# neobotix/neo_mpc_planner2

Measured on AMD Instinct MI355X. Metric: MPC solves/sec (control_steps=3, 500x500 costmap), higher is better.
Workload: dtype f64

## Files before the change

neo_mpc_planner2_amd/csrc/adjoint.h:

```cpp
#pragma once
#include "neo_mpc_device.h"
#include "wave_ops.h"
#include "fast_math.h"
#include "solver_context.h"
#include "costmap.h"
#include "riccati.h"

namespace neo_mpc {
namespace {

template <bool kTame, bool kRiccati, int kFew = 0>
__device__ __forceinline__ void adjoint_by_scans(const SolveArgs& a, const Ctx& c, double* L, bool exact_step, int lane, int n,
                                                 bool& free_path, int& nhops) {
  auto scan = [](double v) { if constexpr (kFew > 0) return wave_scan_few<kFew>(v); else return wave_scan(v); };
  constexpr int kLast = kFew > 0 ? kFew - 1 : 63;
  const DevParams& p = a.p;
  const double* u = L + a.lds.u;
  double* gs = L + a.lds.gs;
  float* RS = reinterpret_cast<float*>(L + a.lds.ric);
  float* ARTF = reinterpret_cast<float*>(L + a.lds.rt);
  const bool on = lane < n;
  const double vx = on ? u[3 * lane] : 0.0, vy = on ? u[3 * lane + 1] : 0.0, w = on ? u[3 * lane + 2] : 0.0;
  const double th = scan(w * p.dt);
  double sn, cs;
  sincos_heading<kTame>(th, &sn, &cs);
  const double ddx = (vx * cs - vy * sn) * p.dt, ddy = (vx * sn + vy * cs) * p.dt;
  const double x = scan(ddx), y = scan(ddy);
  double rt = on ? -2.0 * p.wo_n * (c.tyaw - th) : 0.0;
  if (lane == n - 1) rt += -2.0 * p.wterm_o * (c.fyaw - th);
  const double rx = on ? -2.0 * p.wt_n * (c.cx - x) : 0.0, ry = on ? -2.0 * p.wt_n * (c.cy - y) : 0.0;
  const double px = scan(rx), py = scan(ry);
  const double SX = lane_value(px, kLast) - px + rx, SY = lane_value(py, kLast) - py + ry;
  const double tt = on ? rt - ddy * SX + ddx * SY : 0.0;
  const double pt = scan(tt);
  const double ST = lane_value(pt, kLast) - pt + tt;
  int raw_here = 0;
  bool has_hop = false;
  float hop_x = 0.0f, hop_y = 0.0f;
  if (on) {
    gs[3 * lane] = p.dt * (cs * SX + sn * SY);
    gs[3 * lane + 1] = p.dt * (-sn * SX + cs * SY);
    gs[3 * lane + 2] = p.dt * ST;
    if (kRiccati) {
      float* rs = RS + kRicStage * lane;
      rs[RS_CS] = (float)cs; rs[RS_SN] = (float)sn; rs[RS_PX] = (float)ddx; rs[RS_PY] = (float)ddy;
      double wxx, wxy, wyy, wlx, wly;
      raw_here = edge_stickiness(a, c, L, x, y, cs, sn, wxx, wxy, wyy, wlx, wly, has_hop, hop_x, hop_y);
      rs[RS_WXX] = (float)wxx; rs[RS_WXY] = (float)wxy; rs[RS_WYY] = (float)wyy;
      rs[RS_WLX] = (float)wlx; rs[RS_WLY] = (float)wly;
      rs[RS_SY] = exact_step ? (float)SY : 0.0f;
      ARTF[2 * lane + 1] = exact_step ? (float)SX : 0.0f;
    }
  }
  if (kRiccati) {
    free_path = __ballot(raw_here != 0) == 0ull;
    const unsigned long long hmask = __ballot(has_hop);
    const int rank = __popcll(hmask & ((1ull << lane) - 1ull));
    double* t = L + a.lds.tol;
    if (has_hop && rank < kHopLanes) {
      reinterpret_cast<int*>(t + T_HOP_STAGE)[rank] = lane;
      reinterpret_cast<float*>(t + T_HOP_VEC)[2 * rank] = hop_x;
      reinterpret_cast<float*>(t + T_HOP_VEC)[2 * rank + 1] = hop_y;
    }
    nhops = min(__popcll(hmask), (int)kHopLanes);
    if (lane == 0) reinterpret_cast<int*>(t + T_HOP_STAGE)[kHopLanes] = nhops;
  }
  WAVE_SYNC();
}

template <int kSteps, bool kTame>
__device__ __forceinline__ void adjoint_short_sweep(const SolveArgs& a, const Ctx& c, double* L, bool have_trig, int lane, int n) {
  const DevParams& p = a.p;
  const double* u = L + a.lds.u;
  double* gs = L + a.lds.gs;
  double* ACS = L + a.lds.cs;
  double* ASN = L + a.lds.sn;
  double* ADX = L + a.lds.dxs;
  double* ADY = L + a.lds.dys;
  double* ARX = L + a.lds.rx;
  double* ARY = L + a.lds.ry;
  double* ART = L + a.lds.rt;
  double x = 0.0, y = 0.0, th = 0.0;
#pragma unroll
  for (int i = 0; i < n; ++i) {
    const double vx = u[3 * i], vy = u[3 * i + 1], w = u[3 * i + 2];
    th += w * p.dt;
    double sn, cs;
    if (kSteps && have_trig) { sn = ASN[i]; cs = ACS[i]; }
    else sincos_heading<kTame>(th, &sn, &cs);
    const double ddx = (vx * cs - vy * sn) * p.dt, ddy = (vx * sn + vy * cs) * p.dt;
    x += ddx; y += ddy;
    double rt = -2.0 * p.wo_n * (c.tyaw - th);
    if (i == n - 1) rt += -2.0 * p.wterm_o * (c.fyaw - th);
    if (lane == 0) {
      ACS[i] = cs; ASN[i] = sn; ADX[i] = ddx; ADY[i] = ddy;
      ARX[i] = -2.0 * p.wt_n * (c.cx - x); ARY[i] = -2.0 * p.wt_n * (c.cy - y); ART[i] = rt;
    }
  }
  WAVE_SYNC();
  double SX = 0.0, SY = 0.0, ST = 0.0;
#pragma unroll
  for (int k = n - 1; k >= 0; --k) {
    SX += ARX[k]; SY += ARY[k];
    ST += ART[k] - ADY[k] * SX + ADX[k] * SY;
    if (lane == 0) {
      gs[3 * k] = p.dt * (ACS[k] * SX + ASN[k] * SY);
      gs[3 * k + 1] = p.dt * (-ASN[k] * SX + ACS[k] * SY);
      gs[3 * k + 2] = p.dt * ST;
    }
  }
  WAVE_SYNC();
}

}
}
```

neo_mpc_planner2_amd/csrc/costmap.h:

```cpp
#pragma once
#include <hip/hip_runtime.h>
#include <math.h>
#include <stdint.h>

#include "neo_mpc_device.h"
#include "wave_ops.h"
#include "solver_context.h"
#include "fast_math.h"
#include "solver_rules.h"

namespace neo_mpc {
namespace {

__device__ __forceinline__ int cell_of(double w, double origin, double res, double inv) {
  double t = w - origin;
  double q = t * inv;
  double fl = floor(q);
  if (fabs(q - rint(q)) < 1e-6) fl = floor(t / res);
  int cell;
  asm("v_cvt_i32_f64 %0, %1" : "=v"(cell) : "v"(fl));
  return cell;
}

__device__ __forceinline__ int map_raw(const DevMap& m, int mx, int my) {
  if (mx < -m.border || my < -m.border || mx >= m.size_x + m.border || my >= m.size_y + m.border)
    return 254;
  return m.cells[(long)my * m.pitch + mx];
}

__device__ __forceinline__ int raw_occupancy(int raw) {
  return raw == 0 ? 0 : raw == 253 ? 99 : raw == 254 ? 100 : raw == 255 ? -1 : 1 + (97 * (raw - 1)) / 251;
}
__device__ __forceinline__ double raw_cost(int raw) { return (double)raw_occupancy(raw) / 100.0; }

template <bool kCovered = false>
__device__ __forceinline__ int cell_raw(const SolveArgs& a, const Ctx& c, const double* L, int mx, int my) {
  const unsigned tx = (unsigned)(mx - c.tile_x0), ty = (unsigned)(my - c.tile_y0);
  const int lg = c.tile_geom & 31;
  if (kCovered || ((tx >> lg) == 0u && ty < (unsigned)(c.tile_geom >> 8)))
    return reinterpret_cast<const uint8_t*>(L + a.lds.tile)[(ty << lg) + tx];
  return map_raw(a.map, mx, my);
}

template <bool kCovered = false>
__device__ __forceinline__ double step_term(const SolveArgs& a, const Ctx& c, const double* L, double x, double y) {
  if (c.tile_geom & kTileFree) return L[a.lds.term];
  const double X = c.X0 + (c.c0 * x - c.s0 * y), Y = c.Y0 + (c.s0 * x + c.c0 * y);
  const int mx = cell_of(X, a.map.origin_x, a.map.resolution, a.map.inv_resolution);
  const int my = cell_of(Y, a.map.origin_y, a.map.resolution, a.map.inv_resolution);
  return L[a.lds.term + cell_raw<kCovered>(a, c, L, mx, my)];
}

constexpr double kSticky = NEO_RULE_STICKY, kWall = NEO_RULE_WALL, kStickyDist = NEO_RULE_STICKY_DIST, kWallDist = NEO_RULE_WALL_DIST;
constexpr double kHopMargin = NEO_RULE_HOP_MARGIN;
template <bool kCovered = false>
__device__ __forceinline__ int edge_stickiness(const SolveArgs& a, const Ctx& c, const double* L, double x, double y,
                                               double cs, double sn, double& wxx, double& wxy, double& wyy, double& lx,
                                               double& ly, bool& hop, float& hop_x, float& hop_y) {
  wxx = 0.0; wxy = 0.0; wyy = 0.0; lx = 0.0; ly = 0.0;
  hop = false; hop_x = 0.0f; hop_y = 0.0f;
  if (c.tile_geom & kTileFree) return 0;
  const double X = c.X0 + (c.c0 * x - c.s0 * y), Y = c.Y0 + (c.s0 * x + c.c0 * y);
  const int mx = cell_of(X, a.map.origin_x, a.map.resolution, a.map.inv_resolution);
  const int my = cell_of(Y, a.map.origin_y, a.map.resolution, a.map.inv_resolution);
  const double fx = (X - a.map.origin_x) * a.map.inv_resolution - (double)mx;
  const double fy = (Y - a.map.origin_y) * a.map.inv_resolution - (double)my;
  const int raw_here = cell_raw<kCovered>(a, c, L, mx, my);
  const double here = L[a.lds.term + raw_here];
  const bool far = mx <= -2147483647 || mx >= 2147483646 || my <= -2147483647 || my >= 2147483646;
  if (far) return raw_here;
  const double hop_range = L[a.lds.tol + T_HOP_RANGE];
  const double zone = fmax(kWallDist, hop_range);
  const bool xlo = fx < zone, xhi = 1.0 - fx < zone, ylo = fy < zone, yhi = 1.0 - fy < zone;
  double rx = 0.0, ry = 0.0, pbx = 0.0, pby = 0.0;
  double drop = L[a.lds.tol + T_HOP_DROP], hwx = 0.0, hwy = 0.0;
  if (xlo || xhi) {
    const int raw_n = cell_raw<kCovered>(a, c, L, xlo ? mx - 1 : mx + 1, my);
    const double dist = xlo ? fx : 1.0 - fx, there = L[a.lds.term + raw_n];
    const bool wall = raw_n == 254 && raw_here != 254;
    if (wall) { if (dist < kWallDist) { rx = kWall * 2.0 * a.p.wt_n; pbx = (xlo ? kWallDist - dist : dist - kWallDist) * a.map.resolution; } }
    else if (dist < kStickyDist && there > here) rx = kSticky * 2.0 * a.p.wt_n;
    if (dist < hop_range && here - there > drop) {
      drop = here - there; hop = true;
      hwx = (xlo ? -1.0 : 1.0) * (dist + kHopMargin) * a.map.resolution; hwy = 0.0;
    }
  }
  if (ylo || yhi) {
    const int raw_n = cell_raw<kCovered>(a, c, L, mx, ylo ? my - 1 : my + 1);
    const double dist = ylo ? fy : 1.0 - fy, there = L[a.lds.term + raw_n];
    const bool wall = raw_n == 254 && raw_here != 254;
    if (wall) { if (dist < kWallDist) { ry = kWall * 2.0 * a.p.wt_n; pby = (ylo ? kWallDist - dist : dist - kWallDist) * a.map.resolution; } }
    else if (dist < kStickyDist && there > here) ry = kSticky * 2.0 * a.p.wt_n;
    if (dist < hop_range && here - there > drop) {
      hop = true;
      hwx = 0.0; hwy = (ylo ? -1.0 : 1.0) * (dist + kHopMargin) * a.map.resolution;
    }
  }
  wxx = rx * c.c0 * c.c0 + ry * c.s0 * c.s0;
  wxy = rx * c.c0 * -c.s0 + ry * c.s0 * c.c0;
  wyy = rx * c.s0 * c.s0 + ry * c.c0 * c.c0;
  lx = -(rx * pbx * c.c0 + ry * pby * c.s0);
  ly = -(rx * pbx * -c.s0 + ry * pby * c.c0);
  if (hop) {
    const double hrx = c.c0 * hwx + c.s0 * hwy, hry = -c.s0 * hwx + c.c0 * hwy, idt = rcp_fast(a.p.dt);
    hop_x = (float)((cs * hrx + sn * hry) * idt); hop_y = (float)((-sn * hrx + cs * hry) * idt);
  }
  return raw_here;
}

__device__ double edge_cost(const DevMap& m, double ax, double ay, double bx, double by) {
  int x0 = cell_of(ax, m.origin_x, m.resolution, m.inv_resolution);
  int y0 = cell_of(ay, m.origin_y, m.resolution, m.inv_resolution);
  const int x1 = cell_of(bx, m.origin_x, m.resolution, m.inv_resolution);
  const int y1 = cell_of(by, m.origin_y, m.resolution, m.inv_resolution);
  if (x0 < 0 || y0 < 0 || x0 >= m.size_x || y0 >= m.size_y || x1 < 0 || y1 < 0 || x1 >= m.size_x || y1 >= m.size_y)
    return raw_cost(254);
  const long dx = labs((long)x1 - x0), dy = labs((long)y1 - y0);
  const int sx = x1 >= x0 ? 1 : -1, sy = y1 >= y0 ? 1 : -1;
  long err = dx - dy;
  double worst = -1.0;
  for (long guard = 0; guard <= dx + dy + 1; ++guard) {
    worst = fmax(worst, raw_cost(map_raw(m, x0, y0)));
    if (x0 == x1 && y0 == y1) break;
    long e2 = 2 * err;
    if (e2 > -dy) { err -= dy; x0 += sx; }
    if (e2 < dx) { err += dx; y0 += sy; }
  }
  return worst;
}

__device__ double footprint_cost(const SolveArgs& a, const double* L, uint32_t b, int lane) {
  if (!a.footprints || a.footprint_points == 0) return L[a.lds.prob + P_FOOTPRINT];
  const int np = (int)a.footprint_points;
  const double* pts = a.footprints + (size_t)b * 2 * np;
  double worst = -1.0;
  for (int e = lane; e < np; e += kLanes) {
    int j = (e + 1) % np;
    worst = fmax(worst, edge_cost(a.map, pts[2 * e], pts[2 * e + 1], pts[2 * j], pts[2 * j + 1]));
  }
  return wave_max(worst);
}

}
}
```

neo_mpc_planner2_amd/csrc/feasible_set.h:

```cpp
#pragma once
#include <hip/hip_runtime.h>
#include <math.h>
#include <stdint.h>

#include "neo_mpc_device.h"
#include "fast_math.h"
#include "solver_context.h"

namespace neo_mpc {
namespace {

__device__ __forceinline__ double clampd(double v, double lo, double hi) { return v < lo ? lo : (v > hi ? hi : v); }

template <bool kTame = false>
__device__ __forceinline__ void project_block(const DevParams& p, double& b0, double& b1, double& b2) {
  b2 = fmin(fmax(b2, p.lo[2]), p.hi[2]);
  const double zx = b0, zy = b1, r = p.r;
  if (kTame || p.disc_in_box) {
    const double n2 = zx * zx + zy * zy;
    if (n2 > r * r) { const double sc = r * rsq_fast1(n2); b0 = zx * sc; b1 = zy * sc; }
    return;
  }
  const double px = clampd(zx, p.lo[0], p.hi[0]), py = clampd(zy, p.lo[1], p.hi[1]);
  if (px * px + py * py <= r * r) { b0 = px; b1 = py; return; }
  const double nz = sqrt(zx * zx + zy * zy);
  const double qx = zx * (r / nz), qy = zy * (r / nz);
  if (qx >= p.lo[0] && qx <= p.hi[0] && qy >= p.lo[1] && qy <= p.hi[1]) { b0 = qx; b1 = qy; return; }
  double best = INFINITY, bx = px, by = py;
  for (int e = 0; e < 4; ++e) {
    const double fixed = (e == 0) ? p.lo[0] : (e == 1) ? p.hi[0] : (e == 2) ? p.lo[1] : p.hi[1];
    if (fabs(fixed) > r) continue;
    const double o = sqrt(r * r - fixed * fixed);
    for (int s = -1; s <= 1; s += 2) {
      const double ex = (e < 2) ? fixed : s * o, ey = (e < 2) ? s * o : fixed;
      if (ex < p.lo[0] || ex > p.hi[0] || ey < p.lo[1] || ey > p.hi[1]) continue;
      const double dd = (ex - zx) * (ex - zx) + (ey - zy) * (ey - zy);
      if (dd < best) { best = dd; bx = ex; by = ey; }
    }
  }
  b0 = bx; b1 = by;
}

#define NEO_QN_STEPS                                                                                  \
  1.0, 0.84, 1.19, 0.71, 1.41, 0.59, 1.68, 0.5, 2.0, 0.42, 2.38, 0.35, 2.83, 0.25, 4.0, 0.177,         \
  0.125, 0.088, 0.0625, 0.044, 0.03125, 0.0156, 0.0078, 0.0039, 0.00195, 0.00098, 4.9e-4, 2.4e-4,    \
  1.2e-4, 6e-5, 3e-5, 1.5e-5
__constant__ double kQnSteps[32] = {NEO_QN_STEPS};
constexpr unsigned long long newton_lanes_at_least(double t) {
  constexpr double steps[32] = {NEO_QN_STEPS};
  unsigned long long m = 0;
  for (int l = 32; l < 64; ++l) {
    const double s = l >= 61 ? (double)(1 << (l - 58)) : steps[l - 32];
    if (s >= t) m |= 1ull << l;
  }
  return m;
}
constexpr unsigned long long kNewtonLanes = 0xffffffff00000000ull;

template <bool kLongShots>
__device__ __forceinline__ double lane_scale(int lane) {
  if (kLongShots && lane >= 61) return ldexp(1.0, lane - 58);
  if (lane >= 32) return kQnSteps[lane - 32];
  double s = ldexp(1.0, -12 + (lane >> 1));
  return (lane & 1) ? s * 1.4142135623730951 : s;
}

template <bool kTame = false, bool kRiccati = false>
__device__ __forceinline__ void candidate_block(const SolveArgs& a, const Ctx& c, const double* L, int lane,
                                                double step, double pstep, int i, double& b0, double& b1,
                                                double& b2, int hop_stage = -1, float hop_x = 0.0f, float hop_y = 0.0f) {
  const double* u = L + a.lds.u + 3 * i;
  if (kRiccati && hop_stage >= 0) {
    b0 = u[0]; b1 = u[1]; b2 = u[2];
    if (i == hop_stage) { b0 += (double)hop_x; b1 += (double)hop_y; project_block<kTame>(a.p, b0, b1, b2); }
    return;
  }
  const int* am = reinterpret_cast<const int*>(L + a.lds.mode) + 4 * i;
  const bool near = am[2] != 0;
  if (near && lane >= 32 && (lane & 1)) { b0 = u[0]; b1 = u[1]; b2 = u[2]; return; }
  if (lane < 32 || near) {
    if (lane >= 32) step = pstep;
    if (kRiccati) step *= (double)a.p.n * rcp_fast((double)(a.p.n - i));
    const double* gs = L + a.lds.gs + 3 * i;
    const double e0 = (u[0] - step * gs[0]) - c.v0, e1 = (u[1] - step * gs[1]) - c.v1,
                 e2 = (u[2] - step * gs[2]) - c.v2;
    const double ne2 = e0 * e0 + e1 * e1 + e2 * e2;
    const double sh = (ne2 > 0.0) ? fmax(0.0, 1.0 - step * a.p.wc_n * rsq_fast1(ne2)) : 0.0;
    b0 = c.v0 + sh * e0; b1 = c.v1 + sh * e1; b2 = c.v2 + sh * e2;
  } else {
    const double* d = L + a.lds.d + 3 * i;
    if (kRiccati && am[3]) {
      if (step >= 1.0) { b0 = c.v0; b1 = c.v1; b2 = c.v2; }
      else { b0 = u[0] + step * d[0]; b1 = u[1] + step * d[1]; b2 = u[2] + step * d[2]; }
    } else {
      b0 = u[0] + step * d[0]; b1 = u[1] + step * d[1]; b2 = u[2] + step * d[2];
      const double rl = a.p.r * (1.0 - 1e-12);
      if (!kTame && !a.p.disc_in_box && am[0] == 1 && !(am[1] & 2) && u[0] * u[0] + u[1] * u[1] < rl * rl) {
        const double nxb = L[a.lds.nx + i];
        const double fixed = nxb != 0.0 ? u[0] : u[1];
        const double lim2 = a.p.r * a.p.r - fixed * fixed, lim = lim2 > 0.0 ? sqrt(lim2) * (1.0 - 1e-15) : 0.0;
        if (nxb != 0.0) { b0 = fixed; b1 = clampd(b1, -lim, lim); }
        else { b1 = fixed; b0 = clampd(b0, -lim, lim); }
      }
    }
  }
  project_block<kTame>(a.p, b0, b1, b2);
}

}
}
```

neo_mpc_planner2_amd/csrc/k1_solve.h:

```cpp
#pragma once
#include <hip/hip_runtime.h>
#include <hip/hip_ext.h>
#include <math.h>
#include <stdint.h>
#include <stdlib.h>

#include "neo_mpc_device.h"
#include "wave_ops.h"
#include "fast_math.h"
#include "solver_context.h"
#include "solver_rules.h"
#include "costmap.h"
#include "feasible_set.h"
#include "rollout.h"
#include "riccati.h"
#include "adjoint.h"
#include "tangent_cone.h"
#include "dense_newton.h"
#include "lbfgs.h"
#include "cell_scan.h"
#include "k1_timing.h"

namespace neo_mpc {
namespace {

constexpr int kStallIterations = NEO_RULE_STALL_ITERATIONS;
constexpr int kBlockedRun = NEO_RULE_BLOCKED_RUN;
constexpr double kBlockedStep = NEO_RULE_BLOCKED_STEP;
constexpr double kFinalFracGaussNewton = NEO_RULE_FINAL_FRAC_GN;
constexpr double kWindowStep = NEO_RULE_WINDOW_STEP;
constexpr int kClosingRun = NEO_RULE_CLOSING_RUN;
constexpr int kLateIteration = NEO_RULE_LATE_ITERATION;
constexpr int kNewtonMaxSteps = 8;

constexpr int kRoutedSteps = 3;
constexpr LdsLayout make_routed_stagewise_layout() {
  LdsLayout l = make_lds_layout(kRoutedSteps, 0, true, true);
  constexpr LdsLayout dense = make_lds_layout(kRoutedSteps, 4, false);
  l.tile = dense.tile;
  l.total_bytes = dense.total_bytes;
  return l;
}
static_assert(make_lds_layout(kRoutedSteps, 0, true, true).tile <= make_lds_layout(kRoutedSteps, 4, false).tile,
              "the stage-wise arrays of three stages fit in front of the dense kernel's reach tile");
static_assert(make_lds_layout(kRoutedSteps, 0, true, true).gr == make_lds_layout(kRoutedSteps, 4, false).gr,
              "records, iterate and gradients share their offsets");
template <int kSteps, int kStaticTile, int kLayoutSteps, bool kRouted = false>
__device__ __forceinline__ void fresh_args(SolveArgs& a) {
  auto kp = (const __attribute__((address_space(4))) char*)__builtin_amdgcn_kernarg_segment_ptr();
  asm volatile("" : "+s"(kp));
  a = *(const SolveArgs*)kp;
  if (kRouted) {
    constexpr LdsLayout kLayout = make_routed_stagewise_layout();
    const int tile_w = a.lds.tile_w, tile_h = a.lds.tile_h, reach = a.lds.reach;
    a.lds = kLayout;
    a.lds.tile_w = tile_w; a.lds.tile_h = tile_h; a.lds.reach = reach;
    a.p.n = kRoutedSteps;
  } else if (kSteps || kStaticTile) {
    constexpr LdsLayout kStaticLayout = make_lds_layout(kLayoutSteps, kSteps ? 4 : 0, false);
    const int tile_w = a.lds.tile_w, tile_h = a.lds.tile_h, reach = a.lds.reach;
    a.lds = kStaticLayout;
    a.lds.tile_w = tile_w; a.lds.tile_h = tile_h; a.lds.reach = reach;
    if (kSteps) a.p.n = kSteps;
  }
}
__device__ __forceinline__ void own_loop_params(SolveArgs& a) {
  auto own = [](double& v) { asm volatile("" : "+s"(v)); };
  own(a.p.dt); own(a.p.wt_n); own(a.p.wo_n); own(a.p.wc_n); own(a.p.wterm_o); own(a.p.r);
  own(a.p.lo[2]); own(a.p.hi[2]);
  own(a.map.origin_x); own(a.map.origin_y); own(a.map.resolution); own(a.map.inv_resolution);
}
template <bool kVectorPose>
__device__ __forceinline__ void ctx_from_lds(const SolveArgs& a, const double* L, Ctx& c) {
  const double* P = L + a.lds.prob;
  const double* t = L + a.lds.tol;
  c.cx = lane_value(P[P_CARROT_X], 0); c.cy = lane_value(P[P_CARROT_Y], 0);
  c.tyaw = lane_value(t[T_TYAW], 0); c.fyaw = lane_value(t[T_FYAW], 0);
  c.v0 = lane_value(P[P_VEL], 0); c.v1 = lane_value(P[P_VEL + 1], 0); c.v2 = lane_value(P[P_VEL + 2], 0);
  c.c0 = t[T_C0]; c.s0 = t[T_S0]; c.X0 = P[P_CUR_X]; c.Y0 = P[P_CUR_Y];
  if (kVectorPose) asm volatile("" : "+v"(c.c0), "+v"(c.s0), "+v"(c.X0), "+v"(c.Y0));
  else { c.c0 = lane_value(c.c0, 0); c.s0 = lane_value(c.s0, 0); c.X0 = lane_value(c.X0, 0); c.Y0 = lane_value(c.Y0, 0); }
  const int* ti = reinterpret_cast<const int*>(t + T_TILE);
  c.tile_x0 = uniform_int(ti[0]); c.tile_y0 = uniform_int(ti[1]); c.tile_geom = uniform_int(ti[2]);
  c.konst = 0.0; c.true_yaw = 0.0;
}

struct SolveCarry {
  int flags;
  bool cold;
  bool wall_in_reach;
  double f = INFINITY;
  int it = 0, nfev = 1, status = NEO_MPC_STATUS_MAX_ITER;
};

template <int kSteps, bool kTame, int kStaticTile, int kLayoutSteps>
__device__ __forceinline__ bool solve_setup(double* L, uint32_t b, int lane, SolveCarry& s) {
  constexpr bool kCovered = kStaticTile > 0;
  int flags;
  bool cold = true;
  {
    SolveArgs a;
    fresh_args<kSteps, kStaticTile, kLayoutSteps>(a);
    const DevParams& p = a.p;
    const int n = kSteps ? kSteps : p.n, nv = 3 * n;
    load_records(a, L, b, lane);
    if (uniform_int(reinterpret_cast<const int*>(L + a.lds.prob)[PI_SKIP]) == 1) { skip_instance(a, b, lane); return false; }
    select_map(a.map, L + a.lds.prob);
    flags = reset_and_warm(a, L, b, lane) ? NEO_MPC_FLAG_RESET : 0;
    const double fcost = footprint_cost(a, L, b, lane);
    if (lane == 0) L[a.lds.prob + P_FOOTPRINT] = fcost;
    Ctx c;
    make_ctx_wave(p, a.map, L + a.lds.prob, fcost, c, lane);
    load_tile(a, c, L, lane);
    s.wall_in_reach = (c.tile_geom & kTileWall) != 0;
    if (s.wall_in_reach) flags |= NEO_MPC_FLAG_WALL_IN_REACH;
    if (lane == 0) {
      double* t = L + a.lds.tol;
      t[T_XTOL] = p.xtol; t[T_EARLY] = p.early_tol; t[T_FINAL] = p.final_tol; t[T_FTOL] = p.ftol;
      t[T_STALL] = p.stall_step; t[T_WTOL] = p.wtol; t[T_WTOL_LATE] = p.wtol_late; t[T_KINK] = p.kink_radius;
      t[T_KONST] = c.konst; t[T_TRUE_YAW] = c.true_yaw;
      t[T_HOP_DROP] = p.hop_min_drop; t[T_HOP_RANGE] = p.hop_range;
      t[T_BTOL_MAP] = p.btol_map; t[T_BTOL_FREE] = p.btol_free;
      reinterpret_cast<int*>(t + T_HOP_STAGE)[kHopLanes] = 0;
      t[T_C0] = c.c0; t[T_S0] = c.s0; t[T_TYAW] = c.tyaw; t[T_FYAW] = c.fyaw;
      int* ti = reinterpret_cast<int*>(t + T_TILE);
      ti[0] = c.tile_x0; ti[1] = c.tile_y0; ti[2] = c.tile_geom;
    }
    double* u = L + a.lds.u;
    for (int i = lane; i < n; i += kLanes) project_block<kTame>(p, u[3 * i], u[3 * i + 1], u[3 * i + 2]);
    WAVE_SYNC();
    for (int k = 0; k < nv; ++k) cold = cold && (u[k] == 0.0);
    ctx_from_lds<false>(a, L, c);
    {
      double* S = L + a.lds.state;
      int* Si = reinterpret_cast<int*>(S);
      const bool has_prev = uniform_int(Si[SI_HAS_PREV]) == 1 && !(flags & NEO_MPC_FLAG_RESET);
      WAVE_SYNC();
      if (lane == 0) {
        double q0 = has_prev ? S[S_PREV_U0] : u[nv - 3], q1 = has_prev ? S[S_PREV_U0 + 1] : u[nv - 2], q2 = has_prev ? S[S_PREV_U0 + 2] : u[nv - 1];
        project_block<kTame>(p, q0, q1, q2);
        S[S_PREV_U0] = q0; S[S_PREV_U0 + 1] = q1; S[S_PREV_U0 + 2] = q2;
        Si[SI_HAS_PREV] = 0;
      }
      WAVE_SYNC();
    }
    if (!cold && n > 1 && !(p.compat & kCompatNoUnshift) && p.max_it < kDumpGradient) {
      const double* A0 = L + a.lds.state + S_PREV_U0;
      double ts = 0.0;
      const double fs = rollout_cost<kSteps, kTame, kCovered>(
          a, c, L,
          [&](int i, double& b0, double& b1, double& b2) {
            const double* src = lane == 1 ? (i == 0 ? A0 : u + 3 * (i - 1)) : u + 3 * i;
            b0 = src[0]; b1 = src[1]; b2 = src[2];
          },
          NoRecord(), &ts);
      const double f_warm = lane_value(fs, 0), f_alt = lane_value(fs, 1);
      const bool free_both = lane_value(ts, 0) == 0.0 && lane_value(ts, 1) == 0.0;
      if (f_alt < f_warm && free_both) {
        double v0 = 0.0, v1 = 0.0, v2 = 0.0;
        const int k0 = lane, k1 = lane + kLanes, k2 = lane + 2 * kLanes;
        if (k0 < nv) v0 = k0 >= 3 ? u[k0 - 3] : A0[k0];
        if (k1 < nv) v1 = u[k1 - 3];
        if (k2 < nv) v2 = u[k2 - 3];
        WAVE_SYNC();
        if (k0 < nv) u[k0] = v0;
        if (k1 < nv) u[k1] = v1;
        if (k2 < nv) u[k2] = v2;
      } else if (f_alt < f_warm && lane == 0) {
        reinterpret_cast<int*>(L + a.lds.state)[SI_HAS_PREV] = kAltArmed;
      }
      WAVE_SYNC();
    }
  }
  s.flags = flags; s.cold = cold;
  return true;
}

template <int kMinWavesPerSimd, int kSteps, int kDir, bool kTame, int kStaticTile, int kLayoutSteps, bool kRouted = false>
__device__ __forceinline__ bool solve_search(double* L, uint32_t b, SolveCarry& sc) {
  constexpr bool kCovered = kStaticTile > 0;
  constexpr bool kNewton = kDir == 1;
  constexpr bool kRiccati = kDir == 2;
  constexpr bool kSecond = kDir != 0;
  constexpr bool kBlockedRule = kNewton || kRouted;
  static_assert(!kRiccati || kSteps == 0 || kRouted, "the stage-wise direction: run-time-sized, or the routed kernel's control_steps-3 branch");
  static_assert(!kRouted || (kRiccati && kSteps == kRoutedSteps), "the routed branch is the stage-wise one, three stages in registers");
  constexpr int kFew = (kRiccati && kSteps > 0) ? kSteps : 0;
  constexpr int kNwSteps = !kNewton ? 1 : kSteps ? kSteps : kNewtonMaxSteps;
  constexpr bool kVectorPose = kTame;
  constexpr int kRegSteps = kSteps ? kSteps : 1;
  constexpr int kPairs = kSteps ? 4 : NEO_MPC_MAX_LBFGS_MEMORY;
  double f = sc.f;
  const bool cold = sc.cold;
  int npairs = 0, head = 0, nfev = sc.nfev, it = sc.it, status = sc.status, stall = 0;
  int blocked_run = 0;
  int nblocked = 1;
  double u_term = 0.0;
  double gain1 = INFINITY, gain2 = INFINITY;
  bool final_step = false;
  double alpha = 1.0;
  bool scanned = false;
  int nscans = 0;
  bool scan_only = false;
  auto lane_again = []() {
    int zero;
    asm volatile("v_mov_b32 %0, 0" : "=v"(zero));
    return (int)__builtin_amdgcn_mbcnt_hi(~0u, __builtin_amdgcn_mbcnt_lo(~0u, (unsigned)zero));
  };
  NEO_SEGMENT_DECL;
  NEO_SEGMENT(0);
  for (;;) {
  SolveArgs a;
  fresh_args<kSteps, kStaticTile, kLayoutSteps, kRouted>(a);
  own_loop_params(a);
  select_map(a.map, L + a.lds.prob);
  const DevParams& p = a.p;
  const int n = kSteps ? kSteps : p.n, nv = 3 * n, mem = p.mem;
  double cand[3 * kRegSteps], cand_sn[kRegSteps], cand_cs[kRegSteps];
  bool have_trig = false;
  Ctx c;
  ctx_from_lds<kVectorPose>(a, L, c);
  double* u = L + a.lds.u;
  double* gs = L + a.lds.gs;
  double* gt = L + a.lds.gt;
  double* gr = L + a.lds.gr;
  double* d = L + a.lds.d;
  double* u_prev = L + a.lds.u_prev;
  double* gt_prev = L + a.lds.gt_prev;
  double* u_new = L + a.lds.u_new;
  double* ACS = L + a.lds.cs;
  double* ASN = L + a.lds.sn;
  int* AMODE = reinterpret_cast<int*>(L + a.lds.mode);
  static_assert(2 * 7 >= kNewtonRecord, "Newton records do not fit the step arrays");

  if (!scanned && nscans == 0) {
    const int lane = lane_again();
    for (int i = lane; i < n; i += kLanes) { AMODE[4 * i + 2] = 0; AMODE[4 * i + 3] = 0; }
    if (kRouted && lane == 0) L[a.lds.tol + T_KINK] = p.kink_radius_stagewise;
    alpha = kRiccati ? fmax(1.0, n * 0.125) : 1.0;
    if (kFew && lane == 0) { double* t = L + a.lds.tol; t[T_GAIN1] = INFINITY; t[T_GAIN2] = INFINITY; t[T_ALPHA] = alpha; }
    if (kRiccati && lane == 0) L[a.lds.tol + T_MU] = n > 8 ? (double)(n - 8) * 0.125 : 0.0;
  }
  bool v_feasible = false;
  if (kRiccati) {
    double b0 = c.v0, b1 = c.v1, b2 = c.v2;
    asm volatile("" : "+v"(b0), "+v"(b1), "+v"(b2));
    project_block<kTame>(p, b0, b1, b2);
    v_feasible = b0 == c.v0 && b1 == c.v1 && b2 == c.v2;
  }
  double my_scale;
  {
    int l0 = lane_again();
    my_scale = kRiccati ? 0.0 : lane_scale<kSecond>(l0);
  }
  for (; it < p.max_it && !scan_only; ++it) {
    int lane = lane_again();
    const bool exact_step = kRiccati && nblocked == 0;
    int tol_off = a.lds.tol;
    asm volatile("" : "+s"(tol_off));
    const double* TOL = L + tol_off;
    NEO_PHASE_DECL;
    NEO_PHASE(0);
    constexpr int kVars = 3 * kNwSteps;
    const int nvr = kSteps ? kVars : nv;
    bool free_path = false;
    int nhops = 0;
    float hc[kVars];
    float newton_sol = 0.0f;
    if (kNewton) {
      double hcol[kSteps ? kVars : 1];
      const double hstep = 1e-6, inv_h = 1.0 / hstep;
      double pcs[kNwSteps], psn[kNwSteps];
      double x = 0.0, y = 0.0, th = 0.0;
    #pragma unroll
      for (int i = 0; i < kNwSteps; ++i) {
        if (kSteps || i < n) {
          const double vx = u[3 * i] + (lane == 3 * i ? hstep : 0.0);
          const double vy = u[3 * i + 1] + (lane == 3 * i + 1 ? hstep : 0.0);
          const double w = u[3 * i + 2] + (lane == 3 * i + 2 ? hstep : 0.0);
          th += w * p.dt;
          sincos_heading<kTame>(th, &psn[i], &pcs[i]);
          x += (vx * pcs[i] - vy * psn[i]) * p.dt;
          y += (vx * psn[i] + vy * pcs[i]) * p.dt;
        }
      }
      double SX = 0.0, SY = 0.0, ST = 0.0;
    #pragma unroll
      for (int k = kNwSteps - 1; k >= 0; --k) {
        if (kSteps || k < n) {
          const double vx = u[3 * k] + (lane == 3 * k ? hstep : 0.0);
          const double vy = u[3 * k + 1] + (lane == 3 * k + 1 ? hstep : 0.0);
          const double w = u[3 * k + 2] + (lane == 3 * k + 2 ? hstep : 0.0);
          const double pdx = (vx * pcs[k] - vy * psn[k]) * p.dt, pdy = (vx * psn[k] + vy * pcs[k]) * p.dt;
          double prt = -2.0 * p.wo_n * (c.tyaw - th);
          if (k == n - 1) prt += -2.0 * p.wterm_o * (c.fyaw - th);
          SX += -2.0 * p.wt_n * (c.cx - x); SY += -2.0 * p.wt_n * (c.cy - y);
          ST += prt - pdy * SX + pdx * SY;
          const double g0 = p.dt * (pcs[k] * SX + psn[k] * SY), g1 = p.dt * (-psn[k] * SX + pcs[k] * SY),
                       g2 = p.dt * ST;
          if (kSteps) {
            hcol[3 * k] = g0; hcol[3 * k + 1] = g1; hcol[3 * k + 2] = g2;
          } else {
            const double b0 = lane_value(g0, 63), b1 = lane_value(g1, 63), b2 = lane_value(g2, 63);
            if (lane == 63) { gs[3 * k] = b0; gs[3 * k + 1] = b1; gs[3 * k + 2] = b2; }
            hc[3 * k] = (float)((g0 - b0) * inv_h);
            hc[3 * k + 1] = (float)((g1 - b1) * inv_h);
            hc[3 * k + 2] = (float)((g2 - b2) * inv_h);
          }
          x -= pdx; y -= pdy; th -= w * p.dt;
        } else {
          hc[3 * k] = 0.0f; hc[3 * k + 1] = 0.0f; hc[3 * k + 2] = 0.0f;
        }
      }
      if (kSteps) {
    #pragma unroll
        for (int j = 0; j < kVars; ++j) {
          const double base = lane_value(hcol[j], 63);
          if (lane == 63) gs[j] = base;
          hc[j] = (float)((hcol[j] - base) * inv_h);
        }
      }
      WAVE_SYNC();
    }
    else if (!kSteps || kRiccati) adjoint_by_scans<kTame, kRiccati, kFew>(a, c, L, exact_step, lane, n, free_path, nhops);
    else adjoint_short_sweep<kSteps, kTame>(a, c, L, have_trig, lane, n);
    NEO_PHASE(1);
    const bool my_corner = tangent_cone_pass<kTame, kNewton, kRiccati>(a, c, L, TOL[T_KINK], lane, n);
    WAVE_SYNC();
    const bool corner_any = kSecond && !kTame && __ballot(my_corner) != 0ull && (kRiccati ? free_path : (it > 0 && u_term == 0.0));
    NEO_PHASE(2);
    if (p.max_it == kDumpGradient) {
      for (int k = lane; k < nv; k += kLanes) a.solution[(size_t)b * nv + k] = gt[k];
      return true;
    }
    if (kSecond && it == 0 && cold) {
      if (kRiccati) { for (int k = lane; k < nv; k += kLanes) d[k] = -gr[k]; }
      else if (lane < nvr) d[lane] = -gr[lane];
      if (kRiccati) for (int i = lane; i < n; i += kLanes) AMODE[4 * i + 3] = 0;
      WAVE_SYNC();
    } else if (kRiccati) {
      riccati_prepare(a, c, L, n, lane, v_feasible, (float)TOL[T_MU]);
      WAVE_SYNC();
      if (corner_any) riccati_keep_linear_terms(a, L, n, lane, true);
      auto sweep = [&]() {
        riccati_sweep<float, (kMinWavesPerSimd < 4), kFew>(a, L, n, lane);
        riccati_finish(a, c, L, n, lane);
      };
      sweep();
      if (!kTame && corner_any && repin_corner_blocks<true>(a, L, n, lane)) {
        riccati_keep_linear_terms(a, L, n, lane, false);
        sweep();
      }
    } else if (kNewton) {
      newton_sol = dense_newton_direction<kSteps, kNwSteps, kTame>(a, L, hc, corner_any, lane, n, nvr);
    }
    NEO_PHASE(3);
    if (!kSecond) lbfgs_direction<kSteps, kPairs>(a, L, it, mem, head, npairs, lane, n);
    if (kSecond && it > 0) {
      float dm = 0.0f;
      int anynear = 0;
      if (kRiccati) {
        for (int k = lane; k < nv; k += kLanes) {
          const float v = (float)fabs(d[k]);
          dm = (v == v) ? fmaxf(dm, v) : INFINITY;
          anynear |= (AMODE[4 * (k / 3) + 2] == 1);
        }
      } else if (lane < nvr) { dm = fabsf(newton_sol); anynear = (AMODE[4 * (lane / 3) + 2] == 1); }
      dm = wave_max_f(dm);
      const bool near_any = __ballot(anynear != 0) != 0ull;
      if ((double)dm < TOL[T_EARLY] && !near_any && nhops == 0) { status = NEO_MPC_STATUS_CONVERGED; break; }
      if ((double)dm < ((kRiccati && !exact_step) ? kFinalFracGaussNewton : 1.0) * TOL[T_FINAL] && !near_any) final_step = true;
    }
    NEO_PHASE(4);
    if (p.max_it > kDumpGradient && it == p.max_it - kDumpGradient - 1) {
      for (int k = lane; k < nv; k += kLanes) a.solution[(size_t)b * nv + k] = d[k];
      return true;
    }
    const double lscale = kRiccati ? lane_scale<kSecond>(lane) : my_scale;
    const double alpha_now = kFew ? TOL[T_ALPHA] : alpha;
    const double pstep = alpha_now * lscale;
    const double step = lane < 32 ? pstep : lscale;
    bool took_trial = false;
    double fb = INFINITY, cterm = 0.0;
    int best = 32;
    if (kRiccati && free_path && it > 0) took_trial = riccati_free_space_trial<kTame, kCovered, kFew, kBlockedRule>(a, c, L, n, lane, alpha_now, f, fb, cterm);
    const double* ALT0 = L + a.lds.state + S_PREV_U0;
    bool alt_armed = false;
    if (it == 0) alt_armed = uniform_int(reinterpret_cast<const int*>(L + a.lds.state)[SI_HAS_PREV]) == kAltArmed;
    if (!took_trial) {
    int hop_stage = -1;
    float hop_x = 0.0f, hop_y = 0.0f;
    if (kRiccati && lane >= 1 && lane <= nhops) {
      const double* t = TOL;
      hop_stage = reinterpret_cast<const int*>(t + T_HOP_STAGE)[lane - 1];
      hop_x = reinterpret_cast<const float*>(t + T_HOP_VEC)[2 * (lane - 1)];
      hop_y = reinterpret_cast<const float*>(t + T_HOP_VEC)[2 * (lane - 1) + 1];
    }
    double fc = rollout_cost<kSteps, kTame, kCovered>(
        a, c, L,
        [&](int i, double& b0, double& b1, double& b2) {
          candidate_block<kTame, kRiccati>(a, c, L, lane, step, pstep, i, b0, b1, b2, hop_stage, hop_x, hop_y);
          if (it == 0) {
            asm volatile("");
            if (lane == 0) { b0 = u[3 * i]; b1 = u[3 * i + 1]; b2 = u[3 * i + 2]; }
            if (lane == kAltLane && alt_armed) { const double* src = i == 0 ? ALT0 : u + 3 * (i - 1); b0 = src[0]; b1 = src[1]; b2 = src[2]; }
          }
          if (kSteps) { cand[3 * i] = b0; cand[3 * i + 1] = b1; cand[3 * i + 2] = b2; }
        },
        [&](int i, double sn, double cs) {
          if (kSteps && !kSecond) { cand_sn[i] = sn; cand_cs[i] = cs; }
        }, kBlockedRule ? &cterm : nullptr);
    NEO_PHASE(5);
    if (!(fc == fc)) fc = INFINITY;
    if (it == 0) { f = lane_value(fc, 0); if (kNewton) u_term = lane_value(cterm, 0); }
    fb = fc;
    best = lane;
    wave_argmin(fb, best);
    }
    ++nfev;
    if (!(fb < f)) { status = NEO_MPC_STATUS_CONVERGED; ++it; break; }
    const bool alt_won = alt_armed && best == kAltLane;
    float stepmax = 0.0f;
    if (kSteps && kSecond && !took_trial) {
      if (lane == best) {
#pragma unroll
        for (int k = 0; k < 3 * kRegSteps; ++k) {
          stepmax = fmaxf(stepmax, (float)fabs(cand[k] - u[k]));
          u[k] = cand[k];
        }
      }
      stepmax = __builtin_bit_cast(float, __builtin_amdgcn_readlane(__builtin_bit_cast(int, stepmax), best));
      have_trig = true;
    } else {
      if (kSteps && !kSecond) {
        if (lane == best) {
#pragma unroll
          for (int i = 0; i < kRegSteps; ++i) {
            u_new[3 * i] = cand[3 * i]; u_new[3 * i + 1] = cand[3 * i + 1]; u_new[3 * i + 2] = cand[3 * i + 2];
            ASN[i] = cand_sn[i]; ACS[i] = cand_cs[i];
          }
        }
      } else if (!kSteps && !took_trial) {
        const double bstep = lane_value(step, best), bpstep = lane_value(pstep, best);
        int bhop = -1;
        float bhx = 0.0f, bhy = 0.0f;
        if (kRiccati && best >= 1 && best <= nhops) {
          bhop = reinterpret_cast<const int*>(TOL + T_HOP_STAGE)[best - 1];
          bhx = reinterpret_cast<const float*>(TOL + T_HOP_VEC)[2 * (best - 1)];
          bhy = reinterpret_cast<const float*>(TOL + T_HOP_VEC)[2 * (best - 1) + 1];
        }
        for (int i = lane; i < n; i += kLanes) {
          double b0, b1, b2;
          candidate_block<kTame, kRiccati>(a, c, L, best, bstep, bpstep, i, b0, b1, b2, bhop, bhx, bhy);
          if (alt_won) { const double* src = i == 0 ? ALT0 : u + 3 * (i - 1); b0 = src[0]; b1 = src[1]; b2 = src[2]; }
          u_new[3 * i] = b0; u_new[3 * i + 1] = b1; u_new[3 * i + 2] = b2;
        }
      }
      have_trig = true;
      WAVE_SYNC();
      for (int k = lane; k < nv; k += kLanes) {
        const double nu = u_new[k], ou = u[k];
        stepmax = fmaxf(stepmax, (float)fabs(nu - ou));
        if (!kSecond) { u_prev[k] = ou; gt_prev[k] = gt[k]; }
        u[k] = nu;
      }
      stepmax = wave_max_f(stepmax);
    }
    const double gain = f - fb;
    const double fscale = fmax(1.0, fabs(fb));
    stall = (gain <= TOL[T_FTOL] * fscale || (double)stepmax <= TOL[T_STALL]) ? stall + 1 : 0;
    const bool hop_won = (kRiccati && best >= 1 && best <= nhops) || alt_won;
    nblocked = (best < 32 || lane_value(step, best) < kWindowStep || hop_won) ? nblocked + 1 : 0;
    const bool window_on = !kRiccati || kRouted || nblocked >= 3;
    const double wtol0 = TOL[T_WTOL];
    const double wtol = it >= kLateIteration ? TOL[T_WTOL_LATE] : wtol0;
    const double g1 = kFew ? TOL[T_GAIN1] : gain1, g2 = kFew ? TOL[T_GAIN2] : gain2;
    bool creeping = wtol > 0.0 && gain + g1 + g2 <= wtol * fscale && window_on;
    bool free_now = kRiccati ? free_path : false;
    if (kNewton) free_now = lane_value(cterm, best) == 0.0;
    creeping = creeping || (wtol0 > 0.0 && (double)stepmax <= TOL[T_STALL] && gain <= 0.5 * g1 && g1 <= 0.5 * g2 &&
                            (!free_now || (g2 < INFINITY && gain * gain <= TOL[T_FTOL] * fscale * (g1 - gain))) &&
                            ((kRiccati && !kRouted) ? window_on : nblocked >= kClosingRun));
    bool blocked_stop = false;
    if (kBlockedRule) {
      const double bs = lane_value(step, best);
      blocked_run = (best < 32 || bs < kBlockedStep) ? blocked_run + 1 : 0;
      if (blocked_run >= kBlockedRun) {
        const bool free_rollout = lane_value(cterm, best) == 0.0;
        const double btol = free_rollout ? TOL[T_BTOL_FREE] : TOL[T_BTOL_MAP];
        blocked_stop = gain + g1 + g2 <= btol;
      }
    }
    double* TOLW = L + tol_off;
    if (kFew) { if (lane == 0) { TOLW[T_GAIN2] = g1; TOLW[T_GAIN1] = gain; } }
    else { gain2 = gain1; gain1 = gain; }
    f = fb;
    if (nblocked != 0) final_step = false;
    if (kNewton) u_term = lane_value(cterm, best);
    if (kRiccati && !(it == 0 && cold) && !hop_won) {
      constexpr unsigned long long kNearlyFull = newton_lanes_at_least(0.8), kShort = kNewtonLanes & ~newton_lanes_at_least(0.3);
      const double mu0 = n > 8 ? (double)(n - 8) * 0.125 : 0.0, mu = TOL[T_MU];
      double* mu_slot = L + tol_off + T_MU;
      if ((kNearlyFull >> best) & 1ull) { if (lane == 0) *mu_slot = fmax(0.25 * mu, mu0 * 0.0625); }
      else if (best < 32 || ((kShort >> best) & 1ull)) { if (lane == 0) *mu_slot = fmin(4.0 * mu, 16.0 * mu0); }
    }
    if (best < 32 && !hop_won) {
      const double al = clampd(lane_value(step, best), 1e-6, 1e6);
      if (kFew) { if (lane == 0) TOLW[T_ALPHA] = al; }
      else alpha = al;
    }
    WAVE_SYNC();
    NEO_PHASE(6);
    NEO_PHASE_DUMP();
    if ((double)stepmax < TOL[T_XTOL] || stall >= kStallIterations || creeping || final_step || blocked_stop) { status = NEO_MPC_STATUS_CONVERGED; ++it; break; }
  }

  if (!kSecond || scanned || status != NEO_MPC_STATUS_CONVERGED || p.max_it >= kDumpGradient) break;
  const bool nothing_to_scan = (c.tile_geom & kTileFree) || (kNewton && u_term == 0.0);
  if (nothing_to_scan && nscans == 0) break;
  bool resume = false;
  {
    SolveArgs as;
    fresh_args<kSteps, kStaticTile, kLayoutSteps, kRouted>(as);
    select_map(as.map, L + as.lds.prob);
    Ctx cs;
    ctx_from_lds<false>(as, L, cs);
    int ls = lane_again();
    if (nscans == 0 && ls == 0) L[as.lds.tol + T_FSCAN] = f;
    NEO_SEGMENT_SCAN_BEGIN();
    const bool w = !nothing_to_scan &&
                   cell_scan<kSteps, kTame, kCovered>(as, cs, L, f, kNewton ? &u_term : nullptr, nfev, ls, kSteps ? kSteps : as.p.n);
    NEO_SEGMENT_SCAN_END();
    ++nscans;
    scan_only = w && nscans < NEO_RULE_SCAN_REPEATS;
    if (!scan_only) {
      scanned = true;
      WAVE_SYNC();
      resume = L[as.lds.tol + T_FSCAN] - f > as.p.scan_resume_gain && it < as.p.max_it;
      if (kFew && resume) {
        if (ls == 0) { L[as.lds.tol + T_GAIN1] = INFINITY; L[as.lds.tol + T_GAIN2] = INFINITY; }
        WAVE_SYNC();
      }
    }
  }
  if (scan_only) continue;
  if (!resume) break;
  status = NEO_MPC_STATUS_MAX_ITER; stall = 0; final_step = false; blocked_run = 0; nblocked = 1;
  gain1 = INFINITY; gain2 = INFINITY;
  }
  NEO_SEGMENT(1);
  NEO_SEGMENT_DUMP();
  if (scanned && status == NEO_MPC_STATUS_MAX_ITER) status = NEO_MPC_STATUS_CONVERGED;
  sc.f = f; sc.it = it; sc.nfev = nfev; sc.status = status;
  return false;
}

template <int kSteps, int kStaticTile, int kLayoutSteps>
__device__ __forceinline__ void solve_finish(double* L, uint32_t b, int lane, const SolveCarry& sc) {
  const int flags = sc.flags, status = sc.status, it = sc.it, nfev = sc.nfev;
  double f = sc.f;
  SolveArgs a;
  fresh_args<kSteps, kStaticTile, kLayoutSteps>(a);
  select_map(a.map, L + a.lds.prob);
  const DevParams& p = a.p;
  const int n = kSteps ? kSteps : p.n, nv = 3 * n;
  double* u = L + a.lds.u;
  Ctx c;
  ctx_from_lds<false>(a, L, c);
#ifndef NEO_MPC_PHASE_TIMING
  if (a.solution && p.max_it < kDumpGradient)
    for (int k = lane; k < nv; k += kLanes) a.solution[(size_t)b * nv + k] = u[k];
#endif
  WAVE_SYNC();
  f += L[a.lds.tol + T_KONST];
  c.true_yaw = L[a.lds.tol + T_TRUE_YAW];
  postprocess(a, c, L, b, lane, u, status == NEO_MPC_STATUS_CONVERGED, L[a.lds.prob + P_FOOTPRINT], flags, f, status, it, nfev);
}

template <int kMinWavesPerSimd, int kSteps, int kDir = 0, bool kTame = false, int kStaticTile = 0>
__global__ __launch_bounds__(kLanes, kMinWavesPerSimd) void k_solve(const SolveArgs args) {
  extern __shared__ __align__(16) double Ldyn[];
  constexpr int kLayoutSteps = kSteps ? kSteps : kNewtonMaxSteps;
  constexpr LdsLayout kStaticLayout = make_lds_layout(kLayoutSteps, kSteps ? 4 : 0, false);
  constexpr int kStaticDoubles = kStaticTile ? (kStaticLayout.total_bytes + kStaticTile) / 8 : 2;
  __shared__ __align__(16) double Lstat[kStaticDoubles];
  double* const L = kStaticTile ? Lstat : Ldyn;
  const int lane = threadIdx.x;
  if (blockIdx.x >= args.count) return;
  const uint32_t b = args.order ? (uint32_t)__builtin_amdgcn_readfirstlane((int)args.order[blockIdx.x]) : blockIdx.x;
  if (b >= args.count) return;
  NEO_WAVE_START;
  SolveCarry sc;
  if (!solve_setup<kSteps, kTame, kStaticTile, kLayoutSteps>(L, b, lane, sc)) return;
  if (solve_search<kMinWavesPerSimd, kSteps, kDir, kTame, kStaticTile, kLayoutSteps>(L, b, sc)) return;
  solve_finish<kSteps, kStaticTile, kLayoutSteps>(L, b, lane, sc);
  NEO_WAVE_END_ARGS(args);
}

template <int kMinWavesPerSimd, bool kTame = false, int kStaticTile = 0>
__global__ __launch_bounds__(kLanes, kMinWavesPerSimd) void k_solve_routed(const SolveArgs args) {
  extern __shared__ __align__(16) double Ldyn[];
  constexpr int kSteps = kRoutedSteps;
  constexpr LdsLayout kStaticLayout = make_lds_layout(kSteps, 4, false);
  constexpr int kStaticDoubles = kStaticTile ? (kStaticLayout.total_bytes + kStaticTile) / 8 : 2;
  __shared__ __align__(16) double Lstat[kStaticDoubles];
  double* const L = kStaticTile ? Lstat : Ldyn;
  const int lane = threadIdx.x;
  if (blockIdx.x >= args.count) return;
  const uint32_t b = args.order ? (uint32_t)__builtin_amdgcn_readfirstlane((int)args.order[blockIdx.x]) : blockIdx.x;
  if (b >= args.count) return;
  NEO_WAVE_START;
  SolveCarry sc;
  if (!solve_setup<kSteps, kTame, kStaticTile, kSteps>(L, b, lane, sc)) return;
  if (__builtin_amdgcn_readfirstlane((int)sc.wall_in_reach)) {
    __builtin_amdgcn_s_setprio(3);
    if (solve_search<kMinWavesPerSimd, kSteps, 2, kTame, kStaticTile, kSteps, true>(L, b, sc)) return;
  } else {
    if (solve_search<kMinWavesPerSimd, kSteps, 1, kTame, kStaticTile, kSteps, false>(L, b, sc)) return;
  }
  solve_finish<kSteps, kStaticTile, kSteps>(L, b, lane, sc);
  NEO_WAVE_END_ARGS(args);
}

int solve_variant(const LaunchTuning& t, int fallback) { return t.solve_waves ? t.solve_waves : fallback; }

using SolveKernel = void (*)(const SolveArgs);
void launch_k1(SolveKernel kernel, size_t lds_bytes, const SolveArgs& a, void* stream, void* ev_start, void* ev_stop) {
  const dim3 grid(a.count), block(kLanes);
  hipEvent_t e0 = (hipEvent_t)ev_start, e1 = (hipEvent_t)ev_stop;
  if (e0 || e1) hipExtLaunchKernelGGL(kernel, grid, block, lds_bytes, (hipStream_t)stream, e0, e1, 0, a);
  else hipLaunchKernelGGL(kernel, grid, block, lds_bytes, (hipStream_t)stream, a);
}
#define NEO_K1_BY_WAVES(w, kernel, ...) \
  ((w) == 4 ? (SolveKernel)kernel<4, __VA_ARGS__> : (w) == 3 ? (SolveKernel)kernel<3, __VA_ARGS__> : (SolveKernel)kernel<2, __VA_ARGS__>)

}
}
```

neo_mpc_planner2_amd/csrc/k1_timing.h:

```cpp
#pragma once

#ifdef NEO_MPC_PHASE_TIMING
#ifdef NEO_MPC_SEGMENT_TIMING
#define NEO_SEGMENT_DECL unsigned long long seg_t0 = 0, seg_t1 = 0, seg_scan = 0, seg_scan_at = 0
#define NEO_SEGMENT(k) seg_t##k = wall_clock64()
#define NEO_SEGMENT_SCAN_BEGIN() seg_scan_at = wall_clock64(); seg_scan = seg_scan_at
#define NEO_SEGMENT_SCAN_END() seg_scan = wall_clock64() - seg_scan
#define NEO_SEGMENT_DUMP()                                                                                   \
  {                                                                                                          \
    SolveArgs ad;                                                                                            \
    fresh_args<kSteps, kStaticTile, kLayoutSteps, kRouted>(ad);                                              \
    const int nvd = 3 * ad.p.n;                                                                              \
    if (ad.solution && lane_again() == 0 && nvd >= 9) {                                                      \
      ad.solution[(size_t)b * nvd + 4] = (double)seg_t0; ad.solution[(size_t)b * nvd + 5] = (double)seg_t1;  \
      ad.solution[(size_t)b * nvd + 3] = (double)seg_scan; ad.solution[(size_t)b * nvd + 2] = (double)seg_scan_at; \
    }                                                                                                        \
  }
#else
#define NEO_SEGMENT_DECL
#define NEO_SEGMENT(k)
#define NEO_SEGMENT_SCAN_BEGIN()
#define NEO_SEGMENT_SCAN_END()
#define NEO_SEGMENT_DUMP()
#endif
#define NEO_WAVE_START const unsigned long long wave_t0 = wall_clock64()
#define NEO_WAVE_END_ARGS(args)                                                                     \
  if ((args).solution && lane == 0 && (args).p.n >= 3) {                                            \
    const int nvw = 3 * (args).p.n;                                                                \
    unsigned int hw_id, xcc_id;                                                                    \
    asm volatile("s_getreg_b32 %0, hwreg(HW_REG_HW_ID)" : "=s"(hw_id));                            \
    asm volatile("s_getreg_b32 %0, hwreg(HW_REG_XCC_ID)" : "=s"(xcc_id));                          \
    (args).solution[(size_t)b * nvw + 6] = (double)wave_t0;                                        \
    (args).solution[(size_t)b * nvw + 7] = (double)wall_clock64();                                 \
    (args).solution[(size_t)b * nvw + 8] = (double)hw_id + 4294967296.0 * (double)(xcc_id & 15u);  \
  }
#define NEO_PHASE_DECL long long phase_clock[8]
#define NEO_PHASE(k) phase_clock[k] = clock64()
#define NEO_PHASE_DUMP()                                                                            \
  if (it == 2 && a.solution && lane == 0)                                                          \
    for (int k = 0; k < 6; ++k) a.solution[(size_t)b * nv + k] = (double)(phase_clock[k + 1] - phase_clock[k])
#else
#define NEO_WAVE_START
#define NEO_WAVE_END_ARGS(args)
#define NEO_SEGMENT_DECL
#define NEO_SEGMENT(k)
#define NEO_SEGMENT_SCAN_BEGIN()
#define NEO_SEGMENT_SCAN_END()
#define NEO_SEGMENT_DUMP()
#define NEO_PHASE_DECL
#define NEO_PHASE(k)
#define NEO_PHASE_DUMP()
#endif
```

neo_mpc_planner2_amd/csrc/riccati.h:

```cpp
#pragma once
#include <hip/hip_runtime.h>
#include <math.h>
#include <stdint.h>

#include "neo_mpc_device.h"
#include "wave_ops.h"
#include "fast_math.h"
#include "solver_context.h"
#include "solver_rules.h"
#include "costmap.h"
#include "feasible_set.h"

namespace neo_mpc {
namespace {

enum : int {
  RS_PX = 0, RS_PY, RS_TX, RS_TY,
  RS_WXX, RS_WXY, RS_WYY, RS_FLAGS,
  RS_C00, RS_C01, RS_C02, RS_C11,
  RS_C12, RS_C22, RS_CS, RS_SN,
  RS_GT = 16,
  RS_GS = 19,
  RS_WK = 22,
  RS_WLX = 25, RS_WLY,
  RS_SY = 27,
  RS_GAIN = 16,
  kRicStage = 28
};
enum : int { RC_FREE3 = 0, RC_SLIDE_W, RC_XY, RC_SLIDE, RC_W, RC_NONE, RC_KINK, RF_CASE = 7, RF_KINK_OK = 8 };

typedef float ric_f4 __attribute__((ext_vector_type(4)));

__device__ __forceinline__ float ric_rcp(float x) { return __builtin_amdgcn_rcpf(x); }
__device__ __forceinline__ double ric_rcp(double x) { return rcp_fast(x); }
template <typename T> __device__ __forceinline__ T ric_max(T a, T b) { return a > b ? a : b; }
template <typename T> __device__ __forceinline__ T ric_abs(T a) { return a < (T)0 ? -a : a; }
__device__ __forceinline__ float ric_fma(float a, float b, float c) { return fmaf(a, b, c); }
__device__ __forceinline__ double ric_fma(double a, double b, double c) { return fma(a, b, c); }
template <typename T> __device__ __forceinline__ T ric_pivot(T p, T delta) { return p > delta ? p : ric_max(ric_abs(p), delta); }

__device__ __forceinline__ void riccati_prepare(const SolveArgs& a, const Ctx& c, double* L, int n, int lane,
                                                bool v_feasible, float mu) {
  if (lane >= n) return;
  const DevParams& p = a.p;
  float* rs = reinterpret_cast<float*>(L + a.lds.ric) + kRicStage * lane;
  const int* am = reinterpret_cast<const int*>(L + a.lds.mode) + 4 * lane;
  const double* gt = L + a.lds.gt + 3 * lane;
  const double* gs = L + a.lds.gs + 3 * lane;
  const double* u = L + a.lds.u + 3 * lane;
  const double cs = rs[RS_CS], sn = rs[RS_SN];
  const double idt = rcp_fast(p.dt);
  rs[RS_GT] = (float)((cs * gt[0] - sn * gt[1]) * idt); rs[RS_GT + 1] = (float)((sn * gt[0] + cs * gt[1]) * idt);
  rs[RS_GT + 2] = (float)(gt[2] * idt);
  rs[RS_GS] = (float)((cs * gs[0] - sn * gs[1]) * idt); rs[RS_GS + 1] = (float)((sn * gs[0] + cs * gs[1]) * idt);
  rs[RS_GS + 2] = (float)(gs[2] * idt);
  const double e0 = u[0] - c.v0, e1 = u[1] - c.v1, e2 = u[2] - c.v2;
  rs[RS_WK] = (float)(-(cs * e0 - sn * e1) * p.dt); rs[RS_WK + 1] = (float)(-(sn * e0 + cs * e1) * p.dt);
  rs[RS_WK + 2] = (float)(-e2 * p.dt);
  const double nx = L[a.lds.nx + lane], ny = L[a.lds.ny + lane];
  const double tx = -ny, ty = nx;
  const float rtx = (float)(cs * tx - sn * ty), rty = (float)(sn * tx + cs * ty);
  rs[RS_TX] = rtx; rs[RS_TY] = rty;
  const int near = am[2];
  const int xy = near ? 2 : am[0];
  const bool wfree = !(near || (am[1] & 1));
  const int kase = xy == 0 ? (wfree ? RC_FREE3 : RC_XY) : xy == 1 ? (wfree ? RC_SLIDE_W : RC_SLIDE) : (wfree ? RC_W : RC_NONE);
  const int flags = kase | ((!near && v_feasible) ? RF_KINK_OK : 0);
  rs[RS_FLAGS] = (float)flags;
  float c00 = 0.0f, c01 = 0.0f, c02 = 0.0f, c11 = 0.0f, c12 = 0.0f, c22 = 0.0f;
  if (!near) {
    const float f0 = (float)(cs * e0 - sn * e1), f1 = (float)(sn * e0 + cs * e1), f2 = (float)e2;
    const float fn2 = f0 * f0 + f1 * f1 + f2 * f2;
    const float ine = fn2 > 0.0f ? __builtin_amdgcn_rsqf(fn2) : 0.0f;
    const float i2 = (float)(idt * idt);
    const float sN = (float)p.wc_n * ine * i2, h0 = f0 * ine, h1 = f1 * ine, h2 = f2 * ine;
    const float k2 = reinterpret_cast<const float*>(L + a.lds.rt)[2 * lane] * i2;
    c00 = sN * (1.0f - h0 * h0) + k2 * rtx * rtx; c01 = -sN * h0 * h1 + k2 * rtx * rty; c02 = -sN * h0 * h2;
    c11 = sN * (1.0f - h1 * h1) + k2 * rty * rty; c12 = -sN * h1 * h2; c22 = sN * (1.0f - h2 * h2);
    const float mt = mu * (float)(2.0 * p.wt_n);
    c00 += mt; c11 += mt; c22 += mu * (float)(2.0 * p.wo_n);
  }
  rs[RS_C00] = c00; rs[RS_C01] = c01; rs[RS_C02] = c02; rs[RS_C11] = c11; rs[RS_C12] = c12; rs[RS_C22] = c22;
}

__device__ __forceinline__ void riccati_keep_linear_terms(const SolveArgs& a, double* L, int n, int lane, bool save) {
  ric_f4* rec = reinterpret_cast<ric_f4*>(reinterpret_cast<float*>(L + a.lds.ric) + kRicStage * lane + RS_GAIN);
  ric_f4* keep = reinterpret_cast<ric_f4*>(L + a.lds.keep) + 3 * lane;
  for (int i = lane; i < n; i += kLanes, rec += 7 * kLanes, keep += 3 * kLanes) {
    if (save) { keep[0] = rec[0]; keep[1] = rec[1]; keep[2] = rec[2]; }
    else { rec[0] = keep[0]; rec[1] = keep[1]; rec[2] = keep[2]; }
  }
  WAVE_SYNC();
}

template <typename T, bool kPrefetch = true, int kFew = 0>
__device__ __forceinline__ void riccati_sweep(const SolveArgs& a, double* L, int n, int lane) {
  const DevParams& p = a.p;
  float* RS = static_cast<float*>(__builtin_assume_aligned(reinterpret_cast<float*>(L + a.lds.ric), 16));
  int* AMODE = reinterpret_cast<int*>(L + a.lds.mode);
  double* d = L + a.lds.d;
  const float* ARTF = reinterpret_cast<const float*>(L + a.lds.rt);
  const T w2 = (T)(2.0 * p.wt_n), wo2 = (T)(2.0 * p.wo_n), wterm2 = (T)(2.0 * p.wterm_o);
  const T wc2 = (T)((p.wc_n * p.wc_n) / (p.dt * p.dt));

  T V00 = (T)0.0, V01 = (T)0.0, V02 = (T)0.0, V11 = (T)0.0, V12 = (T)0.0, V22 = (T)0.0, v0 = (T)0.0, v1 = (T)0.0, v2 = (T)0.0;
  ric_f4 r0, r1, r2, r3, r4, r5, r6;
  if (kPrefetch) {
    const ric_f4* R4 = reinterpret_cast<const ric_f4*>(RS + kRicStage * (n - 1));
    r0 = R4[0]; r1 = R4[1]; r2 = R4[2]; r3 = R4[3]; r4 = R4[4]; r5 = R4[5]; r6 = R4[6];
  }
  for (int i = (kFew ? kFew : n) - 1; i >= 0; --i) {
    const bool first = kFew > 0 && i == 0;
    if (!kPrefetch) {
      const ric_f4* R4 = reinterpret_cast<const ric_f4*>(RS + kRicStage * i);
      r0 = R4[0]; r1 = R4[1]; r2 = R4[2]; r3 = R4[3]; r4 = R4[4]; r5 = R4[5]; r6 = R4[6];
    }
    const T px = r0.x, py = r0.y, rtx = r0.z, rty = r0.w;
    const T wxx = r1.x, wxy = r1.y, wyy = r1.z;
    const int flags = __builtin_amdgcn_readfirstlane((int)r1.w);
    const T c00 = r2.x, c01 = r2.y, c02 = r2.z, c11 = r2.w, c12 = r3.x, c22 = r3.y;
    const T gt0 = r4.x, gt1 = r4.y, gt2 = r4.z, gs0 = r4.w, gs1 = r5.x, gs2 = r5.y, e0 = r5.z, e1 = r5.w, e2 = r6.x;
    v0 += (T)r6.y; v1 += (T)r6.z;
    const T sy = (T)r6.w, sx = (T)ARTF[2 * i + 1];
    if (kPrefetch && i > 0) {
      const ric_f4* R4 = reinterpret_cast<const ric_f4*>(RS + kRicStage * (i - 1));
      r0 = R4[0]; r1 = R4[1]; r2 = R4[2]; r3 = R4[3]; r4 = R4[4]; r5 = R4[5]; r6 = R4[6];
    }
    const T S00 = V00 + w2 + wxx, S01 = V01 + wxy, S11 = V11 + w2 + wyy;
    const T S22 = V22 + wo2 + (i == n - 1 ? wterm2 : (T)0.0);
    const T M02 = ric_fma(-py, S00, ric_fma(px, S01, V02));
    const T M12 = ric_fma(-py, S01, ric_fma(px, S11, V12));
    const T M22 = ric_fma(-py, M02, ric_fma(px, M12, ric_fma(-py, V02, ric_fma(px, V12, S22))));
    const T Z02 = M02 + sy, Z12 = M12 - sx, Z22 = M22 - ric_fma(sx, px, sy * py);
    const T z0 = v0, z1 = v1, z2 = ric_fma(-py, v0, ric_fma(px, v1, v2));
    T k0 = (T)0.0, k1 = (T)0.0, k2 = (T)0.0, K00 = (T)0.0, K01 = (T)0.0, K02 = (T)0.0, K10 = (T)0.0, K11 = (T)0.0, K12 = (T)0.0,
      K20 = (T)0.0, K21 = (T)0.0, K22 = (T)0.0;
    bool tokink = false;
    int kase = flags & RF_CASE;
    if (flags & RF_KINK_OK) {
      const T q0 = gs0 + z0 + S00 * e0 + S01 * e1 + Z02 * e2;
      const T q1 = gs1 + z1 + S01 * e0 + S11 * e1 + Z12 * e2;
      const T q2 = gs2 + z2 + Z02 * e0 + Z12 * e1 + Z22 * e2;
      if (__builtin_amdgcn_readfirstlane((int)(q0 * q0 + q1 * q1 + q2 * q2 <= wc2))) { tokink = true; kase = RC_KINK; }
    }
    const T q0 = gt0 + z0, q1 = gt1 + z1, q2 = gt2 + z2;
    switch (kase) {
      case RC_FREE3: {
        const T Q00 = S00 + c00, Q01 = S01 + c01, Q02 = Z02 + c02, Q11 = S11 + c11, Q12 = Z12 + c12, Q22 = Z22 + c22;
        const T delta = ric_max((T)1e-6 * ric_max(ric_abs(Q00), ric_max(ric_abs(Q11), ric_abs(Q22))), (T)1e-30);
        const T d0 = ric_pivot(Q00, delta), i0 = ric_rcp(d0);
        const T l10 = Q01 * i0, l20 = Q02 * i0;
        const T d1 = ric_pivot(Q11 - l10 * Q01, delta), i1 = ric_rcp(d1);
        const T h12 = Q12 - l20 * Q01;
        const T l21 = h12 * i1;
        const T d2 = ric_pivot(Q22 - l20 * Q02 - l21 * h12, delta), i2 = ric_rcp(d2);
#define NEO_RIC_SOLVE3(r0_, r1_, r2_, x0_, x1_, x2_)                                           \
        {                                                                                        \
          const T y0 = -(r0_), y1 = -(r1_) - l10 * y0, y2 = -(r2_) - l20 * y0 - l21 * y1;        \
          x2_ = y2 * i2;                                                                         \
          x1_ = y1 * i1 - l21 * x2_;                                                             \
          x0_ = y0 * i0 - l10 * x1_ - l20 * x2_;                                                 \
        }
        NEO_RIC_SOLVE3(q0, q1, q2, k0, k1, k2)
        if (first) break;
        NEO_RIC_SOLVE3(S00, S01, M02, K00, K10, K20)
        NEO_RIC_SOLVE3(S01, S11, M12, K01, K11, K21)
        NEO_RIC_SOLVE3(Z02, Z12, Z22, K02, K12, K22)
#undef NEO_RIC_SOLVE3
        v0 = z0 + S00 * k0 + S01 * k1 + M02 * k2;
        v1 = z1 + S01 * k0 + S11 * k1 + M12 * k2;
        v2 = z2 + Z02 * k0 + Z12 * k1 + Z22 * k2;
        V00 = S00 + S00 * K00 + S01 * K10 + M02 * K20;
        V01 = S01 + S00 * K01 + S01 * K11 + M02 * K21;
        V02 = M02 + S00 * K02 + S01 * K12 + M02 * K22;
        V11 = S11 + S01 * K01 + S11 * K11 + M12 * K21;
        V12 = M12 + S01 * K02 + S11 * K12 + M12 * K22;
        V22 = Z22 + Z02 * K02 + Z12 * K12 + Z22 * K22;
        break;
      }
      case RC_SLIDE_W:
      case RC_XY: {
        const bool bw = kase == RC_SLIDE_W;
        const T ax = bw ? rtx : (T)1.0, ay = bw ? rty : (T)0.0;
        const T Q00 = S00 + c00, Q01 = S01 + c01, Q11 = S11 + c11;
        const T Qa0 = ax * Q00 + ay * Q01, Qa1 = ax * Q01 + ay * Q11;
        const T haa = Qa0 * ax + Qa1 * ay;
        const T hab = bw ? ax * (Z02 + c02) + ay * (Z12 + c12) : Qa1;
        const T hbb = bw ? Z22 + c22 : Q11;
        const T ga = ax * q0 + ay * q1, gb = bw ? q2 : q1;
        const T Za0 = ax * S00 + ay * S01, Za1 = ax * S01 + ay * S11, Za2 = ax * Z02 + ay * Z12;
        const T Zb0 = bw ? M02 : S01, Zb1 = bw ? M12 : S11, Zb2 = bw ? Z22 : Z12;
        const T delta = ric_max((T)1e-6 * ric_max(ric_abs(haa), ric_abs(hbb)), (T)1e-30);
        const T d0 = ric_pivot(haa, delta), i0 = ric_rcp(d0);
        const T l = hab * i0;
        const T d1 = ric_pivot(hbb - l * hab, delta), i1 = ric_rcp(d1);
        T ka, kb, Ka0, Ka1, Ka2, Kb0, Kb1, Kb2;
#define NEO_RIC_SOLVE2(ra_, rb_, xa_, xb_)                       \
        {                                                          \
          const T y0 = -(ra_), y1 = -(rb_) - l * y0;               \
          xb_ = y1 * i1;                                           \
          xa_ = y0 * i0 - l * xb_;                                 \
        }
        NEO_RIC_SOLVE2(ga, gb, ka, kb)
        if (first) {
          k0 = ax * ka; k1 = ay * ka;
          if (bw) k2 = kb; else k1 = kb;
          break;
        }
        NEO_RIC_SOLVE2(Za0, Zb0, Ka0, Kb0)
        NEO_RIC_SOLVE2(Za1, Zb1, Ka1, Kb1)
        NEO_RIC_SOLVE2(Za2, Zb2, Ka2, Kb2)
#undef NEO_RIC_SOLVE2
        v0 = z0 + Za0 * ka + Zb0 * kb; v1 = z1 + Za1 * ka + Zb1 * kb; v2 = z2 + Za2 * ka + Zb2 * kb;
        V00 = S00 + Za0 * Ka0 + Zb0 * Kb0; V01 = S01 + Za0 * Ka1 + Zb0 * Kb1; V02 = M02 + Za0 * Ka2 + Zb0 * Kb2;
        V11 = S11 + Za1 * Ka1 + Zb1 * Kb1; V12 = M12 + Za1 * Ka2 + Zb1 * Kb2; V22 = Z22 + Za2 * Ka2 + Zb2 * Kb2;
        k0 = ax * ka; k1 = ay * ka; K00 = ax * Ka0; K01 = ax * Ka1; K02 = ax * Ka2; K10 = ay * Ka0; K11 = ay * Ka1; K12 = ay * Ka2;
        if (bw) { k2 = kb; K20 = Kb0; K21 = Kb1; K22 = Kb2; }
        else { k1 = kb; K10 = Kb0; K11 = Kb1; K12 = Kb2; }
        break;
      }
      case RC_SLIDE: {
        const T Q00 = S00 + c00, Q01 = S01 + c01, Q11 = S11 + c11;
        const T haa = (rtx * Q00 + rty * Q01) * rtx + (rtx * Q01 + rty * Q11) * rty;
        const T i0 = -ric_rcp(ric_pivot(haa, ric_max((T)1e-6 * ric_abs(haa), (T)1e-30)));
        const T Za0 = rtx * S00 + rty * S01, Za1 = rtx * S01 + rty * S11, Za2 = rtx * Z02 + rty * Z12;
        const T ka = (rtx * q0 + rty * q1) * i0, Ka0 = Za0 * i0, Ka1 = Za1 * i0, Ka2 = Za2 * i0;
        if (first) { k0 = rtx * ka; k1 = rty * ka; break; }
        v0 = z0 + Za0 * ka; v1 = z1 + Za1 * ka; v2 = z2 + Za2 * ka;
        V00 = S00 + Za0 * Ka0; V01 = S01 + Za0 * Ka1; V02 = M02 + Za0 * Ka2;
        V11 = S11 + Za1 * Ka1; V12 = M12 + Za1 * Ka2; V22 = Z22 + Za2 * Ka2;
        k0 = rtx * ka; k1 = rty * ka; K00 = rtx * Ka0; K01 = rtx * Ka1; K02 = rtx * Ka2; K10 = rty * Ka0; K11 = rty * Ka1; K12 = rty * Ka2;
        break;
      }
      case RC_W: {
        const T hbb = Z22 + c22;
        const T i0 = -ric_rcp(ric_pivot(hbb, ric_max((T)1e-6 * ric_abs(hbb), (T)1e-30)));
        k2 = q2 * i0;
        if (first) break;
        K20 = M02 * i0; K21 = M12 * i0; K22 = Z22 * i0;
        v0 = z0 + M02 * k2; v1 = z1 + M12 * k2; v2 = z2 + Z22 * k2;
        V00 = S00 + M02 * K20; V01 = S01 + M02 * K21; V02 = M02 + M02 * K22;
        V11 = S11 + M12 * K21; V12 = M12 + M12 * K22; V22 = Z22 + Z22 * K22;
        break;
      }
      case RC_KINK:
        k0 = e0; k1 = e1; k2 = e2;
        if (first) break;
        v0 = z0 + S00 * k0 + S01 * k1 + M02 * k2;
        v1 = z1 + S01 * k0 + S11 * k1 + M12 * k2;
        v2 = z2 + Z02 * k0 + Z12 * k1 + Z22 * k2;
        V00 = S00; V01 = S01; V02 = M02; V11 = S11; V12 = M12; V22 = Z22;
        break;
      default:
        v0 = z0; v1 = z1; v2 = z2;
        V00 = S00; V01 = S01; V02 = M02; V11 = S11; V12 = M12; V22 = Z22;
        break;
    }
    if (lane == 0) {
      ric_f4* G4 = reinterpret_cast<ric_f4*>(RS + kRicStage * i + RS_GAIN);
      G4[0] = ric_f4{(float)K00, (float)K01, (float)K02, (float)K10};
      G4[1] = ric_f4{(float)K11, (float)K12, (float)K20, (float)K21};
      G4[2] = ric_f4{(float)K22, (float)k0, (float)k1, (float)k2};
      AMODE[4 * i + 3] = tokink ? 1 : 0;
    }
  }
  WAVE_SYNC();
  T z0 = (T)0.0, z1 = (T)0.0, z2 = (T)0.0;
  for (int i = 0; i < n; ++i) {
    const ric_f4* R4 = reinterpret_cast<const ric_f4*>(RS + kRicStage * i);
    const ric_f4 s0 = R4[0], g0 = R4[4], g1 = R4[5], g2 = R4[6];
    const T w0 = (T)g2.y + (T)g0.x * z0 + (T)g0.y * z1 + (T)g0.z * z2;
    const T w1 = (T)g2.z + (T)g0.w * z0 + (T)g1.x * z1 + (T)g1.y * z2;
    const T w2f = (T)g2.w + (T)g1.z * z0 + (T)g1.w * z1 + (T)g2.x * z2;
    if (lane == 0) { d[3 * i] = (double)w0; d[3 * i + 1] = (double)w1; d[3 * i + 2] = (double)w2f; }
    const T e0 = z0 + w0, e1 = z1 + w1, e2 = z2 + w2f;
    z0 = ric_fma(-(T)s0.y, e2, e0); z1 = ric_fma((T)s0.x, e2, e1); z2 = e2;
  }
  WAVE_SYNC();
}

__device__ __forceinline__ void riccati_finish(const SolveArgs& a, const Ctx& c, double* L, int n, int lane) {
  if (lane < n) {
    const float* rs = reinterpret_cast<const float*>(L + a.lds.ric) + kRicStage * lane;
    const int* am = reinterpret_cast<const int*>(L + a.lds.mode) + 4 * lane;
    double* d = L + a.lds.d + 3 * lane;
    if (am[3]) {
      const double* u = L + a.lds.u + 3 * lane;
      d[0] = c.v0 - u[0]; d[1] = c.v1 - u[1]; d[2] = c.v2 - u[2];
    } else {
      const double cs = rs[RS_CS], sn = rs[RS_SN], idt = rcp_fast(a.p.dt);
      const double w0 = d[0], w1 = d[1], w2 = d[2];
      double d0 = (cs * w0 + sn * w1) * idt, d1 = (-sn * w0 + cs * w1) * idt;
      const int mode = am[2] ? 2 : am[0];
      if (mode == 1) {
        const double nx = L[a.lds.nx + lane], ny = L[a.lds.ny + lane];
        const double dot = d0 * nx + d1 * ny;
        d0 -= dot * nx; d1 -= dot * ny;
      } else if (mode == 2) { d0 = 0.0; d1 = 0.0; }
      d[0] = d0; d[1] = d1; d[2] = (am[2] || (am[1] & 1)) ? 0.0 : w2 * idt;
    }
  }
  WAVE_SYNC();
}

template <bool kTame, bool kCovered, int kFew, bool kWantTerm>
__device__ __forceinline__ bool riccati_free_space_trial(const SolveArgs& a, const Ctx& c, double* L, int n, int lane,
                                                         double alpha_now, double f, double& fb, double& cterm) {
  constexpr double kTrialRatio = NEO_RULE_TRIAL_RATIO;
  const DevParams& p = a.p;
  const double *u = L + a.lds.u, *gr = L + a.lds.gr;
  double* u_new = L + a.lds.u_new;
  bool took_trial = false;
  const bool on = lane < n;
  double b0 = 0.0, b1 = 0.0, b2 = 0.0, g0 = 0.0, g1 = 0.0, g2 = 0.0;
  if (on) {
    candidate_block<kTame, true>(a, c, L, 32, 1.0, alpha_now, lane, b0, b1, b2);
    g0 = gr[3 * lane]; g1 = gr[3 * lane + 1]; g2 = gr[3 * lane + 2];
    u_new[3 * lane] = b0; u_new[3 * lane + 1] = b1; u_new[3 * lane + 2] = b2;
  }
  auto scan = [](double v) { if constexpr (kFew > 0) return wave_scan_few<kFew>(v); else return wave_scan(v); };
  auto sum = [](double v) { if constexpr (kFew > 0) return wave_sum_few<kFew>(v); else return wave_sum(v); };
  const double th = scan(b2 * p.dt);
  double sn, cs;
  sincos_heading<kTame>(th, &sn, &cs);
  const double x = scan((b0 * cs - b1 * sn) * p.dt), y = scan((b0 * sn + b1 * cs) * p.dt);
  double fi = 0.0, pr = 0.0, tm = 0.0;
  if (on) {
    const double dx = c.cx - x, dy = c.cy - y, et = c.tyaw - th;
    const double e0 = c.v0 - b0, e1 = c.v1 - b1, e2 = c.v2 - b2;
    tm = step_term<kCovered>(a, c, L, x, y);
    fi = p.wt_n * (dx * dx + dy * dy) + p.wo_n * (et * et) + p.wc_n * sqrt_fast(e0 * e0 + e1 * e1 + e2 * e2) + tm;
    if (lane == n - 1) { const double ef = c.fyaw - th; fi += p.wterm_o * (ef * ef); }
    pr = -0.5 * (g0 * (b0 - u[3 * lane]) + g1 * (b1 - u[3 * lane + 1]) + g2 * (b2 - u[3 * lane + 2]));
  }
  const double ft = sum(fi), pred = sum(pr);
  if (ft < f && f - ft >= kTrialRatio * pred) {
    took_trial = true; fb = ft;
    if (kWantTerm) cterm = sum(tm);
  }
  WAVE_SYNC();
  return took_trial;
}

}
}
```

neo_mpc_planner2_amd/csrc/tangent_cone.h:

```cpp
#pragma once
#include "neo_mpc_device.h"
#include "fast_math.h"
#include "solver_context.h"
#include "solver_rules.h"
#include "riccati.h"

namespace neo_mpc {
namespace {

constexpr int kNewtonRecord = 13;

template <bool kTame, bool kNewton, bool kRiccati>
__device__ __forceinline__ bool tangent_cone_pass(const SolveArgs& a, const Ctx& c, double* L, double kink_radius, int lane, int n) {
  constexpr bool kSecond = kNewton || kRiccati;
  const DevParams& p = a.p;
  const double* u = L + a.lds.u;
  double* gs = L + a.lds.gs;
  double* gt = L + a.lds.gt;
  double* gr = L + a.lds.gr;
  double* ANX = L + a.lds.nx;
  double* ANY = L + a.lds.ny;
  int* AMODE = reinterpret_cast<int*>(L + a.lds.mode);
  float* NB = reinterpret_cast<float*>(L + a.lds.cs);
  float* ARTF = reinterpret_cast<float*>(L + a.lds.rt);
  bool my_corner = false;
  for (int i = lane; i < n; i += kLanes) {
    const double u0 = u[3 * i], u1 = u[3 * i + 1], u2 = u[3 * i + 2];
    const double g0 = gs[3 * i], g1 = gs[3 * i + 1], g2 = gs[3 * i + 2];
    const double e0 = u0 - c.v0, e1 = u1 - c.v1, e2 = u2 - c.v2;
    const double ne2 = e0 * e0 + e1 * e1 + e2 * e2;
    const double ine = ne2 > 0.0 ? rsq_fast(ne2) : 0.0;
    const double ne = ne2 * ine;
    double t0, t1, t2;
    if (ne2 > 0.0) {
      const double wn = p.wc_n * ine;
      t0 = g0 + wn * e0; t1 = g1 + wn * e1; t2 = g2 + wn * e2;
    } else {
      const double ng2 = g0 * g0 + g1 * g1 + g2 * g2;
      const double sh = (ng2 > p.wc_n * p.wc_n) ? 1.0 - p.wc_n * rsq_fast(ng2) : 0.0;
      t0 = g0 * sh; t1 = g1 * sh; t2 = g2 * sh;
    }
    if (!kRiccati) AMODE[4 * i + 3] = AMODE[4 * i + 2];
    const bool near = ne < kink_radius;
    if (near) { t0 = g0; t1 = g1; t2 = g2; }
    else { gt[3 * i] = t0; gt[3 * i + 1] = t1; gt[3 * i + 2] = t2; }
    const int wfroz = ((u2 <= p.lo[2] && t2 > 0.0) || (u2 >= p.hi[2] && t2 < 0.0)) ? 1 : 0;
    double r0 = t0, r1 = t1;
    double nx0 = 0.0, ny0 = 0.0, nx1 = 0.0, ny1 = 0.0, nx2 = 0.0, ny2 = 0.0;
    bool v0 = false, v1 = false, v2 = false;
    if (!kTame && !p.disc_in_box) {
      constexpr double kRoom = NEO_RULE_CORNER_ROOM;
      if (u0 <= p.lo[0] + kRoom) { nx0 = -1.0; v0 = true; }
      else if (u0 >= p.hi[0] - kRoom) { nx0 = 1.0; v0 = true; }
      if (u1 <= p.lo[1] + kRoom) { ny1 = -1.0; v1 = true; }
      else if (u1 >= p.hi[1] - kRoom) { ny1 = 1.0; v1 = true; }
    }
    const double nvv2 = u0 * u0 + u1 * u1, rlim = p.r * (1.0 - 1e-12);
    if (nvv2 > 0.0 && nvv2 >= rlim * rlim) { const double iv = rsq_fast(nvv2); nx2 = u0 * iv; ny2 = u1 * iv; v2 = true; }
    const double dx = -t0, dy = -t1;
    const double dn0 = nx0 * dx + ny0 * dy, dn1 = nx1 * dx + ny1 * dy, dn2 = nx2 * dx + ny2 * dy;
    int mode = 0, mslot = -1;
    double mnx = 0.0, mny = 0.0, mlam = 0.0;
    if ((v0 && dn0 > 0.0) || (v1 && dn1 > 0.0) || (v2 && dn2 > 0.0)) {
      double bestn = -1.0;
      mode = 2;
#define NEO_TRY_SLIDE(sk, vk, dnk, nxk, nyk, va, nxa, nya, vb, nxb, nyb)                               \
      if (vk && dnk > 0.0) {                                                                         \
        const double px = dx - dnk * nxk, py = dy - dnk * nyk;                                       \
        const double tol = 1e-14 * (fabs(px) + fabs(py));                                            \
        const bool ok = !(va && nxa * px + nya * py > tol) && !(vb && nxb * px + nyb * py > tol);    \
        const double pn = px * px + py * py;                                                         \
        if (ok && pn > bestn) {                                                                      \
          bestn = pn; mode = 1; mnx = nxk; mny = nyk; r0 = -px; r1 = -py; mslot = sk; mlam = dnk;     \
        }                                                                                            \
      }
      NEO_TRY_SLIDE(2, v2, dn2, nx2, ny2, v0, nx0, ny0, v1, nx1, ny1)
      NEO_TRY_SLIDE(0, v0, dn0, nx0, ny0, v1, nx1, ny1, v2, nx2, ny2)
      NEO_TRY_SLIDE(1, v1, dn1, nx1, ny1, v0, nx0, ny0, v2, nx2, ny2)
#undef NEO_TRY_SLIDE
      if (mode == 2) { r0 = 0.0; r1 = 0.0; }
    }
    if (near) {
      const double s2 = wfroz ? 0.0 : t2;
      gs[3 * i] = r0; gs[3 * i + 1] = r1; gs[3 * i + 2] = s2;
      gt[3 * i] = 0.0; gt[3 * i + 1] = 0.0; gt[3 * i + 2] = 0.0;
      gr[3 * i] = 0.0; gr[3 * i + 1] = 0.0; gr[3 * i + 2] = 0.0;
      const int at_rest = (ne2 == 0.0 && r0 * r0 + r1 * r1 + s2 * s2 <= p.wc_n * p.wc_n) ? 2 : 1;
      ANX[i] = 0.0; ANY[i] = 0.0; AMODE[4 * i] = 0; AMODE[4 * i + 1] = 0; AMODE[4 * i + 2] = at_rest;
      if (kNewton) {
#pragma unroll
        for (int k = 0; k < kNewtonRecord; ++k) NB[kNewtonRecord * i + k] = 0.0f;
      }
      if (kRiccati) ARTF[2 * i] = 0.0f;
      continue;
    }
    gr[3 * i] = r0; gr[3 * i + 1] = r1; gr[3 * i + 2] = wfroz ? 0.0 : t2;
    if (kSecond && !kTame && !p.disc_in_box && mode == 1) {
      const double room = NEO_RULE_CORNER_ROOM, rin = p.r - room;
      my_corner = my_corner || (mslot != 0 && (u0 - p.lo[0] <= room || p.hi[0] - u0 <= room)) ||
                  (mslot != 1 && (u1 - p.lo[1] <= room || p.hi[1] - u1 <= room)) || (mslot != 2 && nvv2 >= rin * rin);
    }
    ANX[i] = mnx; ANY[i] = mny; AMODE[4 * i] = mode; AMODE[4 * i + 1] = wfroz | ((mode == 1 && mslot == 2) ? 2 : 0); AMODE[4 * i + 2] = 0;
    if (kNewton) {
      float* nb = NB + kNewtonRecord * i;
      nb[0] = mode == 0 ? 1.0f : mode == 1 ? (float)(1.0 - mnx * mnx) : 0.0f;
      nb[1] = mode == 1 ? (float)(-mnx * mny) : 0.0f;
      nb[2] = mode == 0 ? 1.0f : mode == 1 ? (float)(1.0 - mny * mny) : 0.0f;
      nb[3] = wfroz ? 0.0f : 1.0f;
      const float f0 = (float)e0, f1 = (float)e1, f2 = (float)e2;
      const float fn2 = f0 * f0 + f1 * f1 + f2 * f2;
      const float ine = fn2 > 0.0f ? __builtin_amdgcn_rsqf(fn2) : 0.0f;
      const float sN = (float)p.wc_n * ine, h0 = f0 * ine, h1 = f1 * ine, h2 = f2 * ine;
      const float k2 = (mode == 1 && mslot == 2) ? (float)(mlam * rcp_fast(p.r)) : 0.0f;
      const float tx = -(float)mny, ty = (float)mnx;
      const float c00 = sN * (1.0f - h0 * h0) + k2 * tx * tx, c01 = -sN * h0 * h1 + k2 * tx * ty,
                  c02 = -sN * h0 * h2, c11 = sN * (1.0f - h1 * h1) + k2 * ty * ty, c12 = -sN * h1 * h2,
                  c22 = sN * (1.0f - h2 * h2);
      nb[4] = c00; nb[5] = c01; nb[6] = c02;
      nb[7] = c01; nb[8] = c11; nb[9] = c12;
      nb[10] = c02; nb[11] = c12; nb[12] = c22;
    }
    if (kRiccati) ARTF[2 * i] = (mode == 1 && mslot == 2) ? (float)(mlam * rcp_fast(p.r)) : 0.0f;
  }
  return my_corner;
}

template <bool kRiccati>
__device__ __forceinline__ bool repin_corner_blocks(const SolveArgs& a, double* L, int n, int lane) {
  int* AMODE = reinterpret_cast<int*>(L + a.lds.mode);
  const double* d = L + a.lds.d;
  const double* u = L + a.lds.u;
  double* gr = L + a.lds.gr;
  const DevParams& p = a.p;
  bool any = false;
  for (int i = lane; i < n; i += kLanes) {
    int* am = AMODE + 4 * i;
    if (am[0] != 1 || (kRiccati && am[3])) continue;
    const double u0 = u[3 * i], u1 = u[3 * i + 1], d0 = d[3 * i], d1 = d[3 * i + 1];
    const bool on_disc = (am[1] & 2) != 0, on_x = !on_disc && L[a.lds.nx + i] != 0.0, on_y = !on_disc && !on_x;
    bool blocked = false;
    if (!on_x) blocked = blocked || (d0 != 0.0 && (d0 > 0.0 ? p.hi[0] - u0 : u0 - p.lo[0]) <= NEO_RULE_CORNER_ROOM);
    if (!on_y) blocked = blocked || (d1 != 0.0 && (d1 > 0.0 ? p.hi[1] - u1 : u1 - p.lo[1]) <= NEO_RULE_CORNER_ROOM);
    if (!on_disc) {
      const double rin = p.r - NEO_RULE_CORNER_ROOM;
      blocked = blocked || (d0 * u0 + d1 * u1 > 0.0 && u0 * u0 + u1 * u1 >= rin * rin);
    }
    if (!blocked) continue;
    any = true;
    am[0] = 2; gr[3 * i] = 0.0; gr[3 * i + 1] = 0.0;
    if (kRiccati) {
      float* rs = reinterpret_cast<float*>(L + a.lds.ric) + kRicStage * i;
      const int flags = (int)rs[RS_FLAGS], kase = flags & RF_CASE;
      rs[RS_FLAGS] = (float)((flags & ~RF_CASE) | (kase == RC_SLIDE_W ? RC_W : kase == RC_SLIDE ? RC_NONE : kase));
    } else {
      float* nb = reinterpret_cast<float*>(L + a.lds.cs) + kNewtonRecord * i;
      nb[0] = 0.0f; nb[1] = 0.0f; nb[2] = 0.0f;
    }
  }
  const bool redo = __ballot(any) != 0ull;
  WAVE_SYNC();
  return redo;
}

}
}
```

Baseline: 24.69 million.

## Keep per-stage data in registers across the three-stage Riccati chain

For the three-stage tame Riccati path, the adjoint, tangent-cone and Riccati-prepare passes now carry per-stage values in a register struct. This removes LDS round-trips and several wave syncs between phases. A new unrolled Riccati direction routine keeps gains in registers and computes the direction and its max-norm directly. The change also precomputes neighbour cell lookups in the stickiness pass, caches the per-lane step multipliers in LDS, and hoists rule-word loads. The cost is more register pressure and extra code paths that have to stay consistent with the LDS-based versions.

```diff
diff --git a/neo_mpc_planner2_amd/csrc/adjoint.h b/neo_mpc_planner2_amd/csrc/adjoint.h
--- a/neo_mpc_planner2_amd/csrc/adjoint.h
+++ b/neo_mpc_planner2_amd/csrc/adjoint.h
@@ -9,9 +9,9 @@
 namespace neo_mpc {
 namespace {
 
-template <bool kTame, bool kRiccati, int kFew = 0>
+template <bool kTame, bool kRiccati, int kFew = 0, bool kCovered = false, bool kLocal = false>
 __device__ __forceinline__ void adjoint_by_scans(const SolveArgs& a, const Ctx& c, double* L, bool exact_step, int lane, int n,
-                                                 bool& free_path, int& nhops) {
+                                                 bool& free_path, int& nhops, StageLocal& sl) {
   auto scan = [](double v) { if constexpr (kFew > 0) return wave_scan_few<kFew>(v); else return wave_scan(v); };
   constexpr int kLast = kFew > 0 ? kFew - 1 : 63;
   const DevParams& p = a.p;
@@ -38,14 +38,16 @@
   bool has_hop = false;
   float hop_x = 0.0f, hop_y = 0.0f;
   if (on) {
-    gs[3 * lane] = p.dt * (cs * SX + sn * SY);
-    gs[3 * lane + 1] = p.dt * (-sn * SX + cs * SY);
-    gs[3 * lane + 2] = p.dt * ST;
+    const double g0 = p.dt * (cs * SX + sn * SY), g1 = p.dt * (-sn * SX + cs * SY), g2 = p.dt * ST;
+    gs[3 * lane] = g0;
+    gs[3 * lane + 1] = g1;
+    gs[3 * lane + 2] = g2;
+    if (kLocal) { sl.u0 = vx; sl.u1 = vy; sl.u2 = w; sl.gs0 = g0; sl.gs1 = g1; sl.gs2 = g2; sl.cs = (float)cs; sl.sn = (float)sn; }
     if (kRiccati) {
       float* rs = RS + kRicStage * lane;
       rs[RS_CS] = (float)cs; rs[RS_SN] = (float)sn; rs[RS_PX] = (float)ddx; rs[RS_PY] = (float)ddy;
       double wxx, wxy, wyy, wlx, wly;
-      raw_here = edge_stickiness(a, c, L, x, y, cs, sn, wxx, wxy, wyy, wlx, wly, has_hop, hop_x, hop_y);
+      raw_here = edge_stickiness<kCovered>(a, c, L, x, y, cs, sn, wxx, wxy, wyy, wlx, wly, has_hop, hop_x, hop_y);
       rs[RS_WXX] = (float)wxx; rs[RS_WXY] = (float)wxy; rs[RS_WYY] = (float)wyy;
       rs[RS_WLX] = (float)wlx; rs[RS_WLY] = (float)wly;
       rs[RS_SY] = exact_step ? (float)SY : 0.0f;
@@ -65,7 +67,7 @@
     nhops = min(__popcll(hmask), (int)kHopLanes);
     if (lane == 0) reinterpret_cast<int*>(t + T_HOP_STAGE)[kHopLanes] = nhops;
   }
-  WAVE_SYNC();
+  if (!kLocal) WAVE_SYNC();
 }
 
 template <int kSteps, bool kTame>
diff --git a/neo_mpc_planner2_amd/csrc/costmap.h b/neo_mpc_planner2_amd/csrc/costmap.h
--- a/neo_mpc_planner2_amd/csrc/costmap.h
+++ b/neo_mpc_planner2_amd/csrc/costmap.h
@@ -65,18 +65,24 @@
   const int my = cell_of(Y, a.map.origin_y, a.map.resolution, a.map.inv_resolution);
   const double fx = (X - a.map.origin_x) * a.map.inv_resolution - (double)mx;
   const double fy = (Y - a.map.origin_y) * a.map.inv_resolution - (double)my;
+  const double hop_range = L[a.lds.tol + T_HOP_RANGE], hop_drop = L[a.lds.tol + T_HOP_DROP];
   const int raw_here = cell_raw<kCovered>(a, c, L, mx, my);
+  const bool pre_xlo = fx < 0.5, pre_ylo = fy < 0.5;
+  int raw_px = 0, raw_py = 0;
+  if (kCovered) { raw_px = cell_raw<true>(a, c, L, pre_xlo ? mx - 1 : mx + 1, my); raw_py = cell_raw<true>(a, c, L, mx, pre_ylo ? my - 1 : my + 1); }
   const double here = L[a.lds.term + raw_here];
+  double term_px = 0.0, term_py = 0.0;
+  if (kCovered) { term_px = L[a.lds.term + raw_px]; term_py = L[a.lds.term + raw_py]; }
   const bool far = mx <= -2147483647 || mx >= 2147483646 || my <= -2147483647 || my >= 2147483646;
   if (far) return raw_here;
-  const double hop_range = L[a.lds.tol + T_HOP_RANGE];
   const double zone = fmax(kWallDist, hop_range);
   const bool xlo = fx < zone, xhi = 1.0 - fx < zone, ylo = fy < zone, yhi = 1.0 - fy < zone;
   double rx = 0.0, ry = 0.0, pbx = 0.0, pby = 0.0;
-  double drop = L[a.lds.tol + T_HOP_DROP], hwx = 0.0, hwy = 0.0;
+  double drop = hop_drop, hwx = 0.0, hwy = 0.0;
   if (xlo || xhi) {
-    const int raw_n = cell_raw<kCovered>(a, c, L, xlo ? mx - 1 : mx + 1, my);
-    const double dist = xlo ? fx : 1.0 - fx, there = L[a.lds.term + raw_n];
+    const bool pre = kCovered && xlo == pre_xlo;
+    const int raw_n = pre ? raw_px : cell_raw<kCovered>(a, c, L, xlo ? mx - 1 : mx + 1, my);
+    const double dist = xlo ? fx : 1.0 - fx, there = pre ? term_px : L[a.lds.term + raw_n];
     const bool wall = raw_n == 254 && raw_here != 254;
     if (wall) { if (dist < kWallDist) { rx = kWall * 2.0 * a.p.wt_n; pbx = (xlo ? kWallDist - dist : dist - kWallDist) * a.map.resolution; } }
     else if (dist < kStickyDist && there > here) rx = kSticky * 2.0 * a.p.wt_n;
@@ -86,8 +92,9 @@
     }
   }
   if (ylo || yhi) {
-    const int raw_n = cell_raw<kCovered>(a, c, L, mx, ylo ? my - 1 : my + 1);
-    const double dist = ylo ? fy : 1.0 - fy, there = L[a.lds.term + raw_n];
+    const bool pre = kCovered && ylo == pre_ylo;
+    const int raw_n = pre ? raw_py : cell_raw<kCovered>(a, c, L, mx, ylo ? my - 1 : my + 1);
+    const double dist = ylo ? fy : 1.0 - fy, there = pre ? term_py : L[a.lds.term + raw_n];
     const bool wall = raw_n == 254 && raw_here != 254;
     if (wall) { if (dist < kWallDist) { ry = kWall * 2.0 * a.p.wt_n; pby = (ylo ? kWallDist - dist : dist - kWallDist) * a.map.resolution; } }
     else if (dist < kStickyDist && there > here) ry = kSticky * 2.0 * a.p.wt_n;
diff --git a/neo_mpc_planner2_amd/csrc/feasible_set.h b/neo_mpc_planner2_amd/csrc/feasible_set.h
--- a/neo_mpc_planner2_amd/csrc/feasible_set.h
+++ b/neo_mpc_planner2_amd/csrc/feasible_set.h
@@ -107,5 +107,35 @@
   project_block<kTame>(a.p, b0, b1, b2);
 }
 
+__device__ __forceinline__ void candidate_block_few(const SolveArgs& a, const Ctx& c, const double* L, int lane, double step,
+                                                    double pstep, int i, bool near, bool tokink, double& b0, double& b1,
+                                                    double& b2, int hop_stage, float hop_x, float hop_y) {
+  const double* u = L + a.lds.u + 3 * i;
+  const bool prox = lane < 32 || near;
+  const double* along = L + (prox ? a.lds.gs : a.lds.d) + 3 * i;
+  const double u0 = u[0], u1 = u[1], u2 = u[2];
+  const double s0 = along[0], s1 = along[1], s2 = along[2];
+  if (hop_stage >= 0) {
+    b0 = u0; b1 = u1; b2 = u2;
+    if (i == hop_stage) { b0 += (double)hop_x; b1 += (double)hop_y; project_block<true>(a.p, b0, b1, b2); }
+    return;
+  }
+  if (near && lane >= 32 && (lane & 1)) { b0 = u0; b1 = u1; b2 = u2; return; }
+  if (prox) {
+    if (lane >= 32) step = pstep;
+    step *= (double)a.p.n * rcp_fast((double)(a.p.n - i));
+    const double e0 = (u0 - step * s0) - c.v0, e1 = (u1 - step * s1) - c.v1,
+                 e2 = (u2 - step * s2) - c.v2;
+    const double ne2 = e0 * e0 + e1 * e1 + e2 * e2;
+    const double sh = (ne2 > 0.0) ? fmax(0.0, 1.0 - step * a.p.wc_n * rsq_fast1(ne2)) : 0.0;
+    b0 = c.v0 + sh * e0; b1 = c.v1 + sh * e1; b2 = c.v2 + sh * e2;
+  } else if (tokink && step >= 1.0) {
+    b0 = c.v0; b1 = c.v1; b2 = c.v2;
+  } else {
+    b0 = u0 + step * s0; b1 = u1 + step * s1; b2 = u2 + step * s2;
+  }
+  project_block<true>(a.p, b0, b1, b2);
+}
+
 }
 }
diff --git a/neo_mpc_planner2_amd/csrc/k1_solve.h b/neo_mpc_planner2_amd/csrc/k1_solve.h
--- a/neo_mpc_planner2_amd/csrc/k1_solve.h
+++ b/neo_mpc_planner2_amd/csrc/k1_solve.h
@@ -45,6 +45,9 @@
               "the stage-wise arrays of three stages fit in front of the dense kernel's reach tile");
 static_assert(make_lds_layout(kRoutedSteps, 0, true, true).gr == make_lds_layout(kRoutedSteps, 4, false).gr,
               "records, iterate and gradients share their offsets");
+constexpr int kRoutedStepTable = (make_lds_layout(kRoutedSteps, 0, true, true).keep + 6 * kRoutedSteps + 1) & ~1;
+static_assert(kRoutedStepTable + kLanes <= make_lds_layout(kRoutedSteps, 4, false).tile,
+              "the step multipliers fit between the stage-wise arrays and the reach tile");
 template <int kSteps, int kStaticTile, int kLayoutSteps, bool kRouted = false>
 __device__ __forceinline__ void fresh_args(SolveArgs& a) {
   auto kp = (const __attribute__((address_space(4))) char*)__builtin_amdgcn_kernarg_segment_ptr();
@@ -186,6 +189,7 @@
   static_assert(!kRiccati || kSteps == 0 || kRouted, "the stage-wise direction: run-time-sized, or the routed kernel's control_steps-3 branch");
   static_assert(!kRouted || (kRiccati && kSteps == kRoutedSteps), "the routed branch is the stage-wise one, three stages in registers");
   constexpr int kFew = (kRiccati && kSteps > 0) ? kSteps : 0;
+  constexpr bool kChainLocal = kFew > 0 && kTame;
   constexpr int kNwSteps = !kNewton ? 1 : kSteps ? kSteps : kNewtonMaxSteps;
   constexpr bool kVectorPose = kTame;
   constexpr int kRegSteps = kSteps ? kSteps : 1;
@@ -208,6 +212,7 @@
     return (int)__builtin_amdgcn_mbcnt_hi(~0u, __builtin_amdgcn_mbcnt_lo(~0u, (unsigned)zero));
   };
   NEO_SEGMENT_DECL;
+  NEO_EVENTS_DECL;
   NEO_SEGMENT(0);
   for (;;) {
   SolveArgs a;
@@ -252,6 +257,7 @@
   {
     int l0 = lane_again();
     my_scale = kRiccati ? 0.0 : lane_scale<kSecond>(l0);
+    if (kRouted) L[kRoutedStepTable + l0] = lane_scale<kSecond>(l0);
   }
   for (; it < p.max_it && !scan_only; ++it) {
     int lane = lane_again();
@@ -267,6 +273,9 @@
     int nhops = 0;
     float hc[kVars];
     float newton_sol = 0.0f;
+    StageLocal sl = {};
+    double dl0 = 0.0, dl1 = 0.0, dl2 = 0.0;
+    int dl_near = 0;
     if (kNewton) {
       double hcol[kSteps ? kVars : 1];
       const double hstep = 1e-6, inv_h = 1.0 / hstep;
@@ -322,29 +331,35 @@
       }
       WAVE_SYNC();
     }
-    else if (!kSteps || kRiccati) adjoint_by_scans<kTame, kRiccati, kFew>(a, c, L, exact_step, lane, n, free_path, nhops);
+    else if (!kSteps || kRiccati) adjoint_by_scans<kTame, kRiccati, kFew, kCovered, kChainLocal>(a, c, L, exact_step, lane, n, free_path, nhops, sl);
     else adjoint_short_sweep<kSteps, kTame>(a, c, L, have_trig, lane, n);
     NEO_PHASE(1);
-    const bool my_corner = tangent_cone_pass<kTame, kNewton, kRiccati>(a, c, L, TOL[T_KINK], lane, n);
-    WAVE_SYNC();
+    const bool my_corner = tangent_cone_pass<kTame, kNewton, kRiccati, kChainLocal>(a, c, L, TOL[T_KINK], lane, n, sl);
+    if (!kChainLocal) WAVE_SYNC();
     const bool corner_any = kSecond && !kTame && __ballot(my_corner) != 0ull && (kRiccati ? free_path : (it > 0 && u_term == 0.0));
     NEO_PHASE(2);
     if (p.max_it == kDumpGradient) {
+      if (kChainLocal) WAVE_SYNC();
       for (int k = lane; k < nv; k += kLanes) a.solution[(size_t)b * nv + k] = gt[k];
       return true;
     }
     if (kSecond && it == 0 && cold) {
+      if (kChainLocal) WAVE_SYNC();
       if (kRiccati) { for (int k = lane; k < nv; k += kLanes) d[k] = -gr[k]; }
       else if (lane < nvr) d[lane] = -gr[lane];
       if (kRiccati) for (int i = lane; i < n; i += kLanes) AMODE[4 * i + 3] = 0;
       WAVE_SYNC();
     } else if (kRiccati) {
-      riccati_prepare(a, c, L, n, lane, v_feasible, (float)TOL[T_MU]);
+      riccati_prepare<kChainLocal>(a, c, L, n, lane, v_feasible, (float)TOL[T_MU], sl);
       WAVE_SYNC();
       if (corner_any) riccati_keep_linear_terms(a, L, n, lane, true);
       auto sweep = [&]() {
-        riccati_sweep<float, (kMinWavesPerSimd < 4), kFew>(a, L, n, lane);
-        riccati_finish(a, c, L, n, lane);
+        if constexpr (kFew > 0) {
+          riccati_direction_few<float, kFew>(a, c, L, lane, dl0, dl1, dl2, dl_near);
+        } else {
+          riccati_sweep<float, (kMinWavesPerSimd < 4), kFew>(a, L, n, lane);
+          riccati_finish(a, c, L, n, lane);
+        }
       };
       sweep();
       if (!kTame && corner_any && repin_corner_blocks<true>(a, L, n, lane)) {
@@ -359,7 +374,13 @@
     if (kSecond && it > 0) {
       float dm = 0.0f;
       int anynear = 0;
-      if (kRiccati) {
+      if (kFew) {
+        const float v0 = (float)fabs(dl0), v1 = (float)fabs(dl1), v2 = (float)fabs(dl2);
+        dm = (v0 == v0) ? fmaxf(dm, v0) : INFINITY;
+        dm = (v1 == v1) ? fmaxf(dm, v1) : INFINITY;
+        dm = (v2 == v2) ? fmaxf(dm, v2) : INFINITY;
+        anynear = (dl_near == 1);
+      } else if (kRiccati) {
         for (int k = lane; k < nv; k += kLanes) {
           const float v = (float)fabs(d[k]);
           dm = (v == v) ? fmaxf(dm, v) : INFINITY;
@@ -376,7 +397,7 @@
       for (int k = lane; k < nv; k += kLanes) a.solution[(size_t)b * nv + k] = d[k];
       return true;
     }
-    const double lscale = kRiccati ? lane_scale<kSecond>(lane) : my_scale;
+    const double lscale = kRouted ? L[kRoutedStepTable + lane] : kRiccati ? lane_scale<kSecond>(lane) : my_scale;
     const double alpha_now = kFew ? TOL[T_ALPHA] : alpha;
     const double pstep = alpha_now * lscale;
     const double step = lane < 32 ? pstep : lscale;
@@ -387,6 +408,16 @@
     const double* ALT0 = L + a.lds.state + S_PREV_U0;
     bool alt_armed = false;
     if (it == 0) alt_armed = uniform_int(reinterpret_cast<const int*>(L + a.lds.state)[SI_HAS_PREV]) == kAltArmed;
+    double t_ftol = 0.0, t_stall = 0.0, t_wtol = 0.0, t_wtol_late = 0.0, t_gain1 = 0.0, t_gain2 = 0.0, t_btol_free = 0.0,
+           t_btol_map = 0.0, t_mu = 0.0, t_xtol = 0.0;
+    auto fetch_rule_words = [&]() {
+      if (kFew) {
+        t_ftol = TOL[T_FTOL]; t_stall = TOL[T_STALL]; t_wtol = TOL[T_WTOL]; t_wtol_late = TOL[T_WTOL_LATE];
+        t_gain1 = TOL[T_GAIN1]; t_gain2 = TOL[T_GAIN2]; t_btol_free = TOL[T_BTOL_FREE]; t_btol_map = TOL[T_BTOL_MAP];
+        t_mu = TOL[T_MU]; t_xtol = TOL[T_XTOL];
+      }
+    };
+    auto rule_word = [&](int slot, double fetched) { return kFew ? fetched : TOL[slot]; };
     if (!took_trial) {
     int hop_stage = -1;
     float hop_x = 0.0f, hop_y = 0.0f;
@@ -396,10 +427,21 @@
       hop_x = reinterpret_cast<const float*>(t + T_HOP_VEC)[2 * (lane - 1)];
       hop_y = reinterpret_cast<const float*>(t + T_HOP_VEC)[2 * (lane - 1) + 1];
     }
+    int stage_words = 0;
+    if (kChainLocal) {
+      int w = 0;
+#pragma unroll
+      for (int i = 0; i < kRegSteps; ++i) w |= (AMODE[4 * i + 2] != 0 ? 1 << (2 * i) : 0) | (AMODE[4 * i + 3] != 0 ? 2 << (2 * i) : 0);
+      stage_words = uniform_int(w);
+    }
     double fc = rollout_cost<kSteps, kTame, kCovered>(
         a, c, L,
         [&](int i, double& b0, double& b1, double& b2) {
-          candidate_block<kTame, kRiccati>(a, c, L, lane, step, pstep, i, b0, b1, b2, hop_stage, hop_x, hop_y);
+          if constexpr (kChainLocal)
+            candidate_block_few(a, c, L, lane, step, pstep, i, ((stage_words >> (2 * i)) & 1) != 0, ((stage_words >> (2 * i)) & 2) != 0,
+                                b0, b1, b2, hop_stage, hop_x, hop_y);
+          else
+            candidate_block<kTame, kRiccati>(a, c, L, lane, step, pstep, i, b0, b1, b2, hop_stage, hop_x, hop_y);
           if (it == 0) {
             asm volatile("");
             if (lane == 0) { b0 = u[3 * i]; b1 = u[3 * i + 1]; b2 = u[3 * i + 2]; }
@@ -466,20 +508,23 @@
       }
       stepmax = wave_max_f(stepmax);
     }
+    fetch_rule_words();
     const double gain = f - fb;
     const double fscale = fmax(1.0, fabs(fb));
-    stall = (gain <= TOL[T_FTOL] * fscale || (double)stepmax <= TOL[T_STALL]) ? stall + 1 : 0;
+    stall = (gain <= rule_word(T_FTOL, t_ftol) * fscale || (double)stepmax <= rule_word(T_STALL, t_stall)) ? stall + 1 : 0;
     const bool hop_won = (kRiccati && best >= 1 && best <= nhops) || alt_won;
+    NEO_EVENT(hop, kRiccati && !took_trial && best >= 1 && best <= nhops);
+    NEO_EVENT(trial, took_trial);
     nblocked = (best < 32 || lane_value(step, best) < kWindowStep || hop_won) ? nblocked + 1 : 0;
     const bool window_on = !kRiccati || kRouted || nblocked >= 3;
-    const double wtol0 = TOL[T_WTOL];
-    const double wtol = it >= kLateIteration ? TOL[T_WTOL_LATE] : wtol0;
-    const double g1 = kFew ? TOL[T_GAIN1] : gain1, g2 = kFew ? TOL[T_GAIN2] : gain2;
+    const double wtol0 = rule_word(T_WTOL, t_wtol);
+    const double wtol = it >= kLateIteration ? rule_word(T_WTOL_LATE, t_wtol_late) : wtol0;
+    const double g1 = kFew ? t_gain1 : gain1, g2 = kFew ? t_gain2 : gain2;
     bool creeping = wtol > 0.0 && gain + g1 + g2 <= wtol * fscale && window_on;
     bool free_now = kRiccati ? free_path : false;
     if (kNewton) free_now = lane_value(cterm, best) == 0.0;
-    creeping = creeping || (wtol0 > 0.0 && (double)stepmax <= TOL[T_STALL] && gain <= 0.5 * g1 && g1 <= 0.5 * g2 &&
-                            (!free_now || (g2 < INFINITY && gain * gain <= TOL[T_FTOL] * fscale * (g1 - gain))) &&
+    creeping = creeping || (wtol0 > 0.0 && (double)stepmax <= rule_word(T_STALL, t_stall) && gain <= 0.5 * g1 && g1 <= 0.5 * g2 &&
+                            (!free_now || (g2 < INFINITY && gain * gain <= rule_word(T_FTOL, t_ftol) * fscale * (g1 - gain))) &&
                             ((kRiccati && !kRouted) ? window_on : nblocked >= kClosingRun));
     bool blocked_stop = false;
     if (kBlockedRule) {
@@ -487,7 +532,7 @@
       blocked_run = (best < 32 || bs < kBlockedStep) ? blocked_run + 1 : 0;
       if (blocked_run >= kBlockedRun) {
         const bool free_rollout = lane_value(cterm, best) == 0.0;
-        const double btol = free_rollout ? TOL[T_BTOL_FREE] : TOL[T_BTOL_MAP];
+        const double btol = free_rollout ? rule_word(T_BTOL_FREE, t_btol_free) : rule_word(T_BTOL_MAP, t_btol_map);
         blocked_stop = gain + g1 + g2 <= btol;
       }
     }
@@ -499,7 +544,7 @@
     if (kNewton) u_term = lane_value(cterm, best);
     if (kRiccati && !(it == 0 && cold) && !hop_won) {
       constexpr unsigned long long kNearlyFull = newton_lanes_at_least(0.8), kShort = kNewtonLanes & ~newton_lanes_at_least(0.3);
-      const double mu0 = n > 8 ? (double)(n - 8) * 0.125 : 0.0, mu = TOL[T_MU];
+      const double mu0 = n > 8 ? (double)(n - 8) * 0.125 : 0.0, mu = rule_word(T_MU, t_mu);
       double* mu_slot = L + tol_off + T_MU;
       if ((kNearlyFull >> best) & 1ull) { if (lane == 0) *mu_slot = fmax(0.25 * mu, mu0 * 0.0625); }
       else if (best < 32 || ((kShort >> best) & 1ull)) { if (lane == 0) *mu_slot = fmin(4.0 * mu, 16.0 * mu0); }
@@ -512,7 +557,7 @@
     WAVE_SYNC();
     NEO_PHASE(6);
     NEO_PHASE_DUMP();
-    if ((double)stepmax < TOL[T_XTOL] || stall >= kStallIterations || creeping || final_step || blocked_stop) { status = NEO_MPC_STATUS_CONVERGED; ++it; break; }
+    if ((double)stepmax < rule_word(T_XTOL, t_xtol) || stall >= kStallIterations || creeping || final_step || blocked_stop) { status = NEO_MPC_STATUS_CONVERGED; ++it; break; }
   }
 
   if (!kSecond || scanned || status != NEO_MPC_STATUS_CONVERGED || p.max_it >= kDumpGradient) break;
@@ -545,11 +590,13 @@
   }
   if (scan_only) continue;
   if (!resume) break;
+  NEO_EVENT(resume, true);
   status = NEO_MPC_STATUS_MAX_ITER; stall = 0; final_step = false; blocked_run = 0; nblocked = 1;
   gain1 = INFINITY; gain2 = INFINITY;
   }
   NEO_SEGMENT(1);
   NEO_SEGMENT_DUMP();
+  NEO_EVENTS_DUMP();
   if (scanned && status == NEO_MPC_STATUS_MAX_ITER) status = NEO_MPC_STATUS_CONVERGED;
   sc.f = f; sc.it = it; sc.nfev = nfev; sc.status = status;
   return false;
@@ -567,7 +614,7 @@
   double* u = L + a.lds.u;
   Ctx c;
   ctx_from_lds<false>(a, L, c);
-#ifndef NEO_MPC_PHASE_TIMING
+#if !defined(NEO_MPC_PHASE_TIMING) && !defined(NEO_MPC_EVENT_COUNTS)
   if (a.solution && p.max_it < kDumpGradient)
     for (int k = lane; k < nv; k += kLanes) a.solution[(size_t)b * nv + k] = u[k];
 #endif
diff --git a/neo_mpc_planner2_amd/csrc/k1_timing.h b/neo_mpc_planner2_amd/csrc/k1_timing.h
--- a/neo_mpc_planner2_amd/csrc/k1_timing.h
+++ b/neo_mpc_planner2_amd/csrc/k1_timing.h
@@ -51,3 +51,22 @@
 #define NEO_PHASE(k)
 #define NEO_PHASE_DUMP()
 #endif
+
+#ifdef NEO_MPC_EVENT_COUNTS
+#define NEO_EVENTS_DECL int ev_hop = 0, ev_trial = 0, ev_resume = 0
+#define NEO_EVENT(name, cond) ev_##name += (cond) ? 1 : 0
+#define NEO_EVENTS_DUMP()                                                                           \
+  {                                                                                                 \
+    SolveArgs ae;                                                                                   \
+    fresh_args<kSteps, kStaticTile, kLayoutSteps, kRouted>(ae);                                     \
+    const int nve = 3 * ae.p.n;                                                                     \
+    if (ae.solution && lane_again() == 0) {                                                         \
+      ae.solution[(size_t)b * nve] = (double)ev_hop; ae.solution[(size_t)b * nve + 1] = (double)ev_trial; \
+      ae.solution[(size_t)b * nve + 2] = (double)ev_resume;                                         \
+    }                                                                                               \
+  }
+#else
+#define NEO_EVENTS_DECL
+#define NEO_EVENT(name, cond)
+#define NEO_EVENTS_DUMP()
+#endif
diff --git a/neo_mpc_planner2_amd/csrc/riccati.h b/neo_mpc_planner2_amd/csrc/riccati.h
--- a/neo_mpc_planner2_amd/csrc/riccati.h
+++ b/neo_mpc_planner2_amd/csrc/riccati.h
@@ -39,16 +39,30 @@
 __device__ __forceinline__ double ric_fma(double a, double b, double c) { return fma(a, b, c); }
 template <typename T> __device__ __forceinline__ T ric_pivot(T p, T delta) { return p > delta ? p : ric_max(ric_abs(p), delta); }
 
+struct StageLocal {
+  double u0, u1, u2;
+  double gs0, gs1, gs2;
+  double gt0, gt1, gt2;
+  double nx, ny;
+  float cs, sn, k2;
+  int mode, wfroz, near;
+};
+
+template <bool kLocal = false>
 __device__ __forceinline__ void riccati_prepare(const SolveArgs& a, const Ctx& c, double* L, int n, int lane,
-                                                bool v_feasible, float mu) {
+                                                bool v_feasible, float mu, const StageLocal& sl = StageLocal()) {
   if (lane >= n) return;
   const DevParams& p = a.p;
   float* rs = reinterpret_cast<float*>(L + a.lds.ric) + kRicStage * lane;
-  const int* am = reinterpret_cast<const int*>(L + a.lds.mode) + 4 * lane;
-  const double* gt = L + a.lds.gt + 3 * lane;
-  const double* gs = L + a.lds.gs + 3 * lane;
-  const double* u = L + a.lds.u + 3 * lane;
-  const double cs = rs[RS_CS], sn = rs[RS_SN];
+  const int* amp = reinterpret_cast<const int*>(L + a.lds.mode) + 4 * lane;
+  const double* gtp = L + a.lds.gt + 3 * lane;
+  const double* gsp = L + a.lds.gs + 3 * lane;
+  const double* up = L + a.lds.u + 3 * lane;
+  const double gt[3] = {kLocal ? sl.gt0 : gtp[0], kLocal ? sl.gt1 : gtp[1], kLocal ? sl.gt2 : gtp[2]};
+  const double gs[3] = {kLocal ? sl.gs0 : gsp[0], kLocal ? sl.gs1 : gsp[1], kLocal ? sl.gs2 : gsp[2]};
+  const double u[3] = {kLocal ? sl.u0 : up[0], kLocal ? sl.u1 : up[1], kLocal ? sl.u2 : up[2]};
+  const int am[3] = {kLocal ? sl.mode : amp[0], kLocal ? sl.wfroz : amp[1], kLocal ? sl.near : amp[2]};
+  const double cs = kLocal ? sl.cs : rs[RS_CS], sn = kLocal ? sl.sn : rs[RS_SN];
   const double idt = rcp_fast(p.dt);
   rs[RS_GT] = (float)((cs * gt[0] - sn * gt[1]) * idt); rs[RS_GT + 1] = (float)((sn * gt[0] + cs * gt[1]) * idt);
   rs[RS_GT + 2] = (float)(gt[2] * idt);
@@ -57,7 +71,7 @@
   const double e0 = u[0] - c.v0, e1 = u[1] - c.v1, e2 = u[2] - c.v2;
   rs[RS_WK] = (float)(-(cs * e0 - sn * e1) * p.dt); rs[RS_WK + 1] = (float)(-(sn * e0 + cs * e1) * p.dt);
   rs[RS_WK + 2] = (float)(-e2 * p.dt);
-  const double nx = L[a.lds.nx + lane], ny = L[a.lds.ny + lane];
+  const double nx = kLocal ? sl.nx : L[a.lds.nx + lane], ny = kLocal ? sl.ny : L[a.lds.ny + lane];
   const double tx = -ny, ty = nx;
   const float rtx = (float)(cs * tx - sn * ty), rty = (float)(sn * tx + cs * ty);
   rs[RS_TX] = rtx; rs[RS_TY] = rty;
@@ -74,7 +88,7 @@
     const float ine = fn2 > 0.0f ? __builtin_amdgcn_rsqf(fn2) : 0.0f;
     const float i2 = (float)(idt * idt);
     const float sN = (float)p.wc_n * ine * i2, h0 = f0 * ine, h1 = f1 * ine, h2 = f2 * ine;
-    const float k2 = reinterpret_cast<const float*>(L + a.lds.rt)[2 * lane] * i2;
+    const float k2 = (kLocal ? sl.k2 : reinterpret_cast<const float*>(L + a.lds.rt)[2 * lane]) * i2;
     c00 = sN * (1.0f - h0 * h0) + k2 * rtx * rtx; c01 = -sN * h0 * h1 + k2 * rtx * rty; c02 = -sN * h0 * h2;
     c11 = sN * (1.0f - h1 * h1) + k2 * rty * rty; c12 = -sN * h1 * h2; c22 = sN * (1.0f - h2 * h2);
     const float mt = mu * (float)(2.0 * p.wt_n);
@@ -91,6 +105,162 @@
     else { rec[0] = keep[0]; rec[1] = keep[1]; rec[2] = keep[2]; }
   }
   WAVE_SYNC();
+}
+
+template <typename T> struct RicGains {
+  T K00 = (T)0.0, K01 = (T)0.0, K02 = (T)0.0, K10 = (T)0.0, K11 = (T)0.0, K12 = (T)0.0, K20 = (T)0.0, K21 = (T)0.0, K22 = (T)0.0;
+  T k0 = (T)0.0, k1 = (T)0.0, k2 = (T)0.0;
+  bool tokink = false;
+};
+template <typename T> struct RicValue {
+  T V00 = (T)0.0, V01 = (T)0.0, V02 = (T)0.0, V11 = (T)0.0, V12 = (T)0.0, V22 = (T)0.0, v0 = (T)0.0, v1 = (T)0.0, v2 = (T)0.0;
+};
+template <typename T> struct RicWeights { T w2, wo2, wterm2, wc2; };
+constexpr int kRicGainsInRegisters = 2;
+
+template <typename T>
+__device__ __forceinline__ void riccati_stage(const ric_f4& r0, const ric_f4& r1, const ric_f4& r2, const ric_f4& r3,
+                                              const ric_f4& r4, const ric_f4& r5, const ric_f4& r6, T sx, bool last, bool first,
+                                              const RicWeights<T>& wts, RicValue<T>& val, RicGains<T>& g) {
+  const T w2 = wts.w2, wo2 = wts.wo2, wterm2 = wts.wterm2, wc2 = wts.wc2;
+  T &V00 = val.V00, &V01 = val.V01, &V02 = val.V02, &V11 = val.V11, &V12 = val.V12, &V22 = val.V22, &v0 = val.v0, &v1 = val.v1, &v2 = val.v2;
+  const T px = r0.x, py = r0.y, rtx = r0.z, rty = r0.w;
+  const T wxx = r1.x, wxy = r1.y, wyy = r1.z;
+  const int flags = __builtin_amdgcn_readfirstlane((int)r1.w);
+  const T c00 = r2.x, c01 = r2.y, c02 = r2.z, c11 = r2.w, c12 = r3.x, c22 = r3.y;
+  const T gt0 = r4.x, gt1 = r4.y, gt2 = r4.z, gs0 = r4.w, gs1 = r5.x, gs2 = r5.y, e0 = r5.z, e1 = r5.w, e2 = r6.x;
+  v0 += (T)r6.y; v1 += (T)r6.z;
+  const T sy = (T)r6.w;
+  const T S00 = V00 + w2 + wxx, S01 = V01 + wxy, S11 = V11 + w2 + wyy;
+  const T S22 = V22 + wo2 + (last ? wterm2 : (T)0.0);
+  const T M02 = ric_fma(-py, S00, ric_fma(px, S01, V02));
+  const T M12 = ric_fma(-py, S01, ric_fma(px, S11, V12));
+  const T M22 = ric_fma(-py, M02, ric_fma(px, M12, ric_fma(-py, V02, ric_fma(px, V12, S22))));
+  const T Z02 = M02 + sy, Z12 = M12 - sx, Z22 = M22 - ric_fma(sx, px, sy * py);
+  const T z0 = v0, z1 = v1, z2 = ric_fma(-py, v0, ric_fma(px, v1, v2));
+  T &k0 = g.k0, &k1 = g.k1, &k2 = g.k2, &K00 = g.K00, &K01 = g.K01, &K02 = g.K02, &K10 = g.K10, &K11 = g.K11, &K12 = g.K12,
+    &K20 = g.K20, &K21 = g.K21, &K22 = g.K22;
+  bool& tokink = g.tokink;
+  int kase = flags & RF_CASE;
+  if (flags & RF_KINK_OK) {
+    const T q0 = gs0 + z0 + S00 * e0 + S01 * e1 + Z02 * e2;
+    const T q1 = gs1 + z1 + S01 * e0 + S11 * e1 + Z12 * e2;
+    const T q2 = gs2 + z2 + Z02 * e0 + Z12 * e1 + Z22 * e2;
+    if (__builtin_amdgcn_readfirstlane((int)(q0 * q0 + q1 * q1 + q2 * q2 <= wc2))) { tokink = true; kase = RC_KINK; }
+  }
+  const T q0 = gt0 + z0, q1 = gt1 + z1, q2 = gt2 + z2;
+  switch (kase) {
+    case RC_FREE3: {
+      const T Q00 = S00 + c00, Q01 = S01 + c01, Q02 = Z02 + c02, Q11 = S11 + c11, Q12 = Z12 + c12, Q22 = Z22 + c22;
+      const T delta = ric_max((T)1e-6 * ric_max(ric_abs(Q00), ric_max(ric_abs(Q11), ric_abs(Q22))), (T)1e-30);
+      const T d0 = ric_pivot(Q00, delta), i0 = ric_rcp(d0);
+      const T l10 = Q01 * i0, l20 = Q02 * i0;
+      const T d1 = ric_pivot(Q11 - l10 * Q01, delta), i1 = ric_rcp(d1);
+      const T h12 = Q12 - l20 * Q01;
+      const T l21 = h12 * i1;
+      const T d2 = ric_pivot(Q22 - l20 * Q02 - l21 * h12, delta), i2 = ric_rcp(d2);
+#define NEO_RIC_SOLVE3(r0_, r1_, r2_, x0_, x1_, x2_)                                           \
+      {                                                                                        \
+        const T y0 = -(r0_), y1 = -(r1_) - l10 * y0, y2 = -(r2_) - l20 * y0 - l21 * y1;        \
+        x2_ = y2 * i2;                                                                         \
+        x1_ = y1 * i1 - l21 * x2_;                                                             \
+        x0_ = y0 * i0 - l10 * x1_ - l20 * x2_;                                                 \
+      }
+      NEO_RIC_SOLVE3(q0, q1, q2, k0, k1, k2)
+      if (first) break;
+      NEO_RIC_SOLVE3(S00, S01, M02, K00, K10, K20)
+      NEO_RIC_SOLVE3(S01, S11, M12, K01, K11, K21)
+      NEO_RIC_SOLVE3(Z02, Z12, Z22, K02, K12, K22)
+#undef NEO_RIC_SOLVE3
+      v0 = z0 + S00 * k0 + S01 * k1 + M02 * k2;
+      v1 = z1 + S01 * k0 + S11 * k1 + M12 * k2;
+      v2 = z2 + Z02 * k0 + Z12 * k1 + Z22 * k2;
+      V00 = S00 + S00 * K00 + S01 * K10 + M02 * K20;
+      V01 = S01 + S00 * K01 + S01 * K11 + M02 * K21;
+      V02 = M02 + S00 * K02 + S01 * K12 + M02 * K22;
+      V11 = S11 + S01 * K01 + S11 * K11 + M12 * K21;
+      V12 = M12 + S01 * K02 + S11 * K12 + M12 * K22;
+      V22 = Z22 + Z02 * K02 + Z12 * K12 + Z22 * K22;
+      break;
+    }
+    case RC_SLIDE_W:
+    case RC_XY: {
+      const bool bw = kase == RC_SLIDE_W;
+      const T ax = bw ? rtx : (T)1.0, ay = bw ? rty : (T)0.0;
+      const T Q00 = S00 + c00, Q01 = S01 + c01, Q11 = S11 + c11;
+      const T Qa0 = ax * Q00 + ay * Q01, Qa1 = ax * Q01 + ay * Q11;
+      const T haa = Qa0 * ax + Qa1 * ay;
+      const T hab = bw ? ax * (Z02 + c02) + ay * (Z12 + c12) : Qa1;
+      const T hbb = bw ? Z22 + c22 : Q11;
+      const T ga = ax * q0 + ay * q1, gb = bw ? q2 : q1;
+      const T Za0 = ax * S00 + ay * S01, Za1 = ax * S01 + ay * S11, Za2 = ax * Z02 + ay * Z12;
+      const T Zb0 = bw ? M02 : S01, Zb1 = bw ? M12 : S11, Zb2 = bw ? Z22 : Z12;
+      const T delta = ric_max((T)1e-6 * ric_max(ric_abs(haa), ric_abs(hbb)), (T)1e-30);
+      const T d0 = ric_pivot(haa, delta), i0 = ric_rcp(d0);
+      const T l = hab * i0;
+      const T d1 = ric_pivot(hbb - l * hab, delta), i1 = ric_rcp(d1);
+      T ka, kb, Ka0, Ka1, Ka2, Kb0, Kb1, Kb2;
+#define NEO_RIC_SOLVE2(ra_, rb_, xa_, xb_)                       \
+      {                                                          \
+        const T y0 = -(ra_), y1 = -(rb_) - l * y0;               \
+        xb_ = y1 * i1;                                           \
+        xa_ = y0 * i0 - l * xb_;                                 \
+      }
+      NEO_RIC_SOLVE2(ga, gb, ka, kb)
+      if (first) {
+        k0 = ax * ka; k1 = ay * ka;
+        if (bw) k2 = kb; else k1 = kb;
+        break;
+      }
+      NEO_RIC_SOLVE2(Za0, Zb0, Ka0, Kb0)
+      NEO_RIC_SOLVE2(Za1, Zb1, Ka1, Kb1)
+      NEO_RIC_SOLVE2(Za2, Zb2, Ka2, Kb2)
+#undef NEO_RIC_SOLVE2
+      v0 = z0 + Za0 * ka + Zb0 * kb; v1 = z1 + Za1 * ka + Zb1 * kb; v2 = z2 + Za2 * ka + Zb2 * kb;
+      V00 = S00 + Za0 * Ka0 + Zb0 * Kb0; V01 = S01 + Za0 * Ka1 + Zb0 * Kb1; V02 = M02 + Za0 * Ka2 + Zb0 * Kb2;
+      V11 = S11 + Za1 * Ka1 + Zb1 * Kb1; V12 = M12 + Za1 * Ka2 + Zb1 * Kb2; V22 = Z22 + Za2 * Ka2 + Zb2 * Kb2;
+      k0 = ax * ka; k1 = ay * ka; K00 = ax * Ka0; K01 = ax * Ka1; K02 = ax * Ka2; K10 = ay * Ka0; K11 = ay * Ka1; K12 = ay * Ka2;
+      if (bw) { k2 = kb; K20 = Kb0; K21 = Kb1; K22 = Kb2; }
+      else { k1 = kb; K10 = Kb0; K11 = Kb1; K12 = Kb2; }
+      break;
+    }
+    case RC_SLIDE: {
+      const T Q00 = S00 + c00, Q01 = S01 + c01, Q11 = S11 + c11;
+      const T haa = (rtx * Q00 + rty * Q01) * rtx + (rtx * Q01 + rty * Q11) * rty;
+      const T i0 = -ric_rcp(ric_pivot(haa, ric_max((T)1e-6 * ric_abs(haa), (T)1e-30)));
+      const T Za0 = rtx * S00 + rty * S01, Za1 = rtx * S01 + rty * S11, Za2 = rtx * Z02 + rty * Z12;
+      const T ka = (rtx * q0 + rty * q1) * i0, Ka0 = Za0 * i0, Ka1 = Za1 * i0, Ka2 = Za2 * i0;
+      if (first) { k0 = rtx * ka; k1 = rty * ka; break; }
+      v0 = z0 + Za0 * ka; v1 = z1 + Za1 * ka; v2 = z2 + Za2 * ka;
+      V00 = S00 + Za0 * Ka0; V01 = S01 + Za0 * Ka1; V02 = M02 + Za0 * Ka2;
+      V11 = S11 + Za1 * Ka1; V12 = M12 + Za1 * Ka2; V22 = Z22 + Za2 * Ka2;
+      k0 = rtx * ka; k1 = rty * ka; K00 = rtx * Ka0; K01 = rtx * Ka1; K02 = rtx * Ka2; K10 = rty * Ka0; K11 = rty * Ka1; K12 = rty * Ka2;
+      break;
+    }
+    case RC_W: {
+      const T hbb = Z22 + c22;
+      const T i0 = -ric_rcp(ric_pivot(hbb, ric_max((T)1e-6 * ric_abs(hbb), (T)1e-30)));
+      k2 = q2 * i0;
+      if (first) break;
+      K20 = M02 * i0; K21 = M12 * i0; K22 = Z22 * i0;
+      v0 = z0 + M02 * k2; v1 = z1 + M12 * k2; v2 = z2 + Z22 * k2;
+      V00 = S00 + M02 * K20; V01 = S01 + M02 * K21; V02 = M02 + M02 * K22;
+      V11 = S11 + M12 * K21; V12 = M12 + M12 * K22; V22 = Z22 + Z22 * K22;
+      break;
+    }
+    case RC_KINK:
+      k0 = e0; k1 = e1; k2 = e2;
+      if (first) break;
+      v0 = z0 + S00 * k0 + S01 * k1 + M02 * k2;
+      v1 = z1 + S01 * k0 + S11 * k1 + M12 * k2;
+      v2 = z2 + Z02 * k0 + Z12 * k1 + Z22 * k2;
+      V00 = S00; V01 = S01; V02 = M02; V11 = S11; V12 = M12; V22 = Z22;
+      break;
+    default:
+      v0 = z0; v1 = z1; v2 = z2;
+      V00 = S00; V01 = S01; V02 = M02; V11 = S11; V12 = M12; V22 = Z22;
+      break;
+  }
 }
 
 template <typename T, bool kPrefetch = true, int kFew = 0>
@@ -100,10 +270,9 @@
   int* AMODE = reinterpret_cast<int*>(L + a.lds.mode);
   double* d = L + a.lds.d;
   const float* ARTF = reinterpret_cast<const float*>(L + a.lds.rt);
-  const T w2 = (T)(2.0 * p.wt_n), wo2 = (T)(2.0 * p.wo_n), wterm2 = (T)(2.0 * p.wterm_o);
-  const T wc2 = (T)((p.wc_n * p.wc_n) / (p.dt * p.dt));
-
-  T V00 = (T)0.0, V01 = (T)0.0, V02 = (T)0.0, V11 = (T)0.0, V12 = (T)0.0, V22 = (T)0.0, v0 = (T)0.0, v1 = (T)0.0, v2 = (T)0.0;
+  const RicWeights<T> wts{(T)(2.0 * p.wt_n), (T)(2.0 * p.wo_n), (T)(2.0 * p.wterm_o), (T)((p.wc_n * p.wc_n) / (p.dt * p.dt))};
+
+  RicValue<T> val;
   ric_f4 r0, r1, r2, r3, r4, r5, r6;
   if (kPrefetch) {
     const ric_f4* R4 = reinterpret_cast<const ric_f4*>(RS + kRicStage * (n - 1));
@@ -115,153 +284,20 @@
       const ric_f4* R4 = reinterpret_cast<const ric_f4*>(RS + kRicStage * i);
       r0 = R4[0]; r1 = R4[1]; r2 = R4[2]; r3 = R4[3]; r4 = R4[4]; r5 = R4[5]; r6 = R4[6];
     }
-    const T px = r0.x, py = r0.y, rtx = r0.z, rty = r0.w;
-    const T wxx = r1.x, wxy = r1.y, wyy = r1.z;
-    const int flags = __builtin_amdgcn_readfirstlane((int)r1.w);
-    const T c00 = r2.x, c01 = r2.y, c02 = r2.z, c11 = r2.w, c12 = r3.x, c22 = r3.y;
-    const T gt0 = r4.x, gt1 = r4.y, gt2 = r4.z, gs0 = r4.w, gs1 = r5.x, gs2 = r5.y, e0 = r5.z, e1 = r5.w, e2 = r6.x;
-    v0 += (T)r6.y; v1 += (T)r6.z;
-    const T sy = (T)r6.w, sx = (T)ARTF[2 * i + 1];
+    const ric_f4 q0 = r0, q1 = r1, q2 = r2, q3 = r3, q4 = r4, q5 = r5, q6 = r6;
+    const T sx = (T)ARTF[2 * i + 1];
     if (kPrefetch && i > 0) {
       const ric_f4* R4 = reinterpret_cast<const ric_f4*>(RS + kRicStage * (i - 1));
       r0 = R4[0]; r1 = R4[1]; r2 = R4[2]; r3 = R4[3]; r4 = R4[4]; r5 = R4[5]; r6 = R4[6];
     }
-    const T S00 = V00 + w2 + wxx, S01 = V01 + wxy, S11 = V11 + w2 + wyy;
-    const T S22 = V22 + wo2 + (i == n - 1 ? wterm2 : (T)0.0);
-    const T M02 = ric_fma(-py, S00, ric_fma(px, S01, V02));
-    const T M12 = ric_fma(-py, S01, ric_fma(px, S11, V12));
-    const T M22 = ric_fma(-py, M02, ric_fma(px, M12, ric_fma(-py, V02, ric_fma(px, V12, S22))));
-    const T Z02 = M02 + sy, Z12 = M12 - sx, Z22 = M22 - ric_fma(sx, px, sy * py);
-    const T z0 = v0, z1 = v1, z2 = ric_fma(-py, v0, ric_fma(px, v1, v2));
-    T k0 = (T)0.0, k1 = (T)0.0, k2 = (T)0.0, K00 = (T)0.0, K01 = (T)0.0, K02 = (T)0.0, K10 = (T)0.0, K11 = (T)0.0, K12 = (T)0.0,
-      K20 = (T)0.0, K21 = (T)0.0, K22 = (T)0.0;
-    bool tokink = false;
-    int kase = flags & RF_CASE;
-    if (flags & RF_KINK_OK) {
-      const T q0 = gs0 + z0 + S00 * e0 + S01 * e1 + Z02 * e2;
-      const T q1 = gs1 + z1 + S01 * e0 + S11 * e1 + Z12 * e2;
-      const T q2 = gs2 + z2 + Z02 * e0 + Z12 * e1 + Z22 * e2;
-      if (__builtin_amdgcn_readfirstlane((int)(q0 * q0 + q1 * q1 + q2 * q2 <= wc2))) { tokink = true; kase = RC_KINK; }
-    }
-    const T q0 = gt0 + z0, q1 = gt1 + z1, q2 = gt2 + z2;
-    switch (kase) {
-      case RC_FREE3: {
-        const T Q00 = S00 + c00, Q01 = S01 + c01, Q02 = Z02 + c02, Q11 = S11 + c11, Q12 = Z12 + c12, Q22 = Z22 + c22;
-        const T delta = ric_max((T)1e-6 * ric_max(ric_abs(Q00), ric_max(ric_abs(Q11), ric_abs(Q22))), (T)1e-30);
-        const T d0 = ric_pivot(Q00, delta), i0 = ric_rcp(d0);
-        const T l10 = Q01 * i0, l20 = Q02 * i0;
-        const T d1 = ric_pivot(Q11 - l10 * Q01, delta), i1 = ric_rcp(d1);
-        const T h12 = Q12 - l20 * Q01;
-        const T l21 = h12 * i1;
-        const T d2 = ric_pivot(Q22 - l20 * Q02 - l21 * h12, delta), i2 = ric_rcp(d2);
-#define NEO_RIC_SOLVE3(r0_, r1_, r2_, x0_, x1_, x2_)                                           \
-        {                                                                                        \
-          const T y0 = -(r0_), y1 = -(r1_) - l10 * y0, y2 = -(r2_) - l20 * y0 - l21 * y1;        \
-          x2_ = y2 * i2;                                                                         \
-          x1_ = y1 * i1 - l21 * x2_;                                                             \
-          x0_ = y0 * i0 - l10 * x1_ - l20 * x2_;                                                 \
-        }
-        NEO_RIC_SOLVE3(q0, q1, q2, k0, k1, k2)
-        if (first) break;
-        NEO_RIC_SOLVE3(S00, S01, M02, K00, K10, K20)
-        NEO_RIC_SOLVE3(S01, S11, M12, K01, K11, K21)
-        NEO_RIC_SOLVE3(Z02, Z12, Z22, K02, K12, K22)
-#undef NEO_RIC_SOLVE3
-        v0 = z0 + S00 * k0 + S01 * k1 + M02 * k2;
-        v1 = z1 + S01 * k0 + S11 * k1 + M12 * k2;
-        v2 = z2 + Z02 * k0 + Z12 * k1 + Z22 * k2;
-        V00 = S00 + S00 * K00 + S01 * K10 + M02 * K20;
-        V01 = S01 + S00 * K01 + S01 * K11 + M02 * K21;
-        V02 = M02 + S00 * K02 + S01 * K12 + M02 * K22;
-        V11 = S11 + S01 * K01 + S11 * K11 + M12 * K21;
-        V12 = M12 + S01 * K02 + S11 * K12 + M12 * K22;
-        V22 = Z22 + Z02 * K02 + Z12 * K12 + Z22 * K22;
-        break;
-      }
-      case RC_SLIDE_W:
-      case RC_XY: {
-        const bool bw = kase == RC_SLIDE_W;
-        const T ax = bw ? rtx : (T)1.0, ay = bw ? rty : (T)0.0;
-        const T Q00 = S00 + c00, Q01 = S01 + c01, Q11 = S11 + c11;
-        const T Qa0 = ax * Q00 + ay * Q01, Qa1 = ax * Q01 + ay * Q11;
-        const T haa = Qa0 * ax + Qa1 * ay;
-        const T hab = bw ? ax * (Z02 + c02) + ay * (Z12 + c12) : Qa1;
-        const T hbb = bw ? Z22 + c22 : Q11;
-        const T ga = ax * q0 + ay * q1, gb = bw ? q2 : q1;
-        const T Za0 = ax * S00 + ay * S01, Za1 = ax * S01 + ay * S11, Za2 = ax * Z02 + ay * Z12;
-        const T Zb0 = bw ? M02 : S01, Zb1 = bw ? M12 : S11, Zb2 = bw ? Z22 : Z12;
-        const T delta = ric_max((T)1e-6 * ric_max(ric_abs(haa), ric_abs(hbb)), (T)1e-30);
-        const T d0 = ric_pivot(haa, delta), i0 = ric_rcp(d0);
-        const T l = hab * i0;
-        const T d1 = ric_pivot(hbb - l * hab, delta), i1 = ric_rcp(d1);
-        T ka, kb, Ka0, Ka1, Ka2, Kb0, Kb1, Kb2;
-#define NEO_RIC_SOLVE2(ra_, rb_, xa_, xb_)                       \
-        {                                                          \
-          const T y0 = -(ra_), y1 = -(rb_) - l * y0;               \
-          xb_ = y1 * i1;                                           \
-          xa_ = y0 * i0 - l * xb_;                                 \
-        }
-        NEO_RIC_SOLVE2(ga, gb, ka, kb)
-        if (first) {
-          k0 = ax * ka; k1 = ay * ka;
-          if (bw) k2 = kb; else k1 = kb;
-          break;
-        }
-        NEO_RIC_SOLVE2(Za0, Zb0, Ka0, Kb0)
-        NEO_RIC_SOLVE2(Za1, Zb1, Ka1, Kb1)
-        NEO_RIC_SOLVE2(Za2, Zb2, Ka2, Kb2)
-#undef NEO_RIC_SOLVE2
-        v0 = z0 + Za0 * ka + Zb0 * kb; v1 = z1 + Za1 * ka + Zb1 * kb; v2 = z2 + Za2 * ka + Zb2 * kb;
-        V00 = S00 + Za0 * Ka0 + Zb0 * Kb0; V01 = S01 + Za0 * Ka1 + Zb0 * Kb1; V02 = M02 + Za0 * Ka2 + Zb0 * Kb2;
-        V11 = S11 + Za1 * Ka1 + Zb1 * Kb1; V12 = M12 + Za1 * Ka2 + Zb1 * Kb2; V22 = Z22 + Za2 * Ka2 + Zb2 * Kb2;
-        k0 = ax * ka; k1 = ay * ka; K00 = ax * Ka0; K01 = ax * Ka1; K02 = ax * Ka2; K10 = ay * Ka0; K11 = ay * Ka1; K12 = ay * Ka2;
-        if (bw) { k2 = kb; K20 = Kb0; K21 = Kb1; K22 = Kb2; }
-        else { k1 = kb; K10 = Kb0; K11 = Kb1; K12 = Kb2; }
-        break;
-      }
-      case RC_SLIDE: {
-        const T Q00 = S00 + c00, Q01 = S01 + c01, Q11 = S11 + c11;
-        const T haa = (rtx * Q00 + rty * Q01) * rtx + (rtx * Q01 + rty * Q11) * rty;
-        const T i0 = -ric_rcp(ric_pivot(haa, ric_max((T)1e-6 * ric_abs(haa), (T)1e-30)));
-        const T Za0 = rtx * S00 + rty * S01, Za1 = rtx * S01 + rty * S11, Za2 = rtx * Z02 + rty * Z12;
-        const T ka = (rtx * q0 + rty * q1) * i0, Ka0 = Za0 * i0, Ka1 = Za1 * i0, Ka2 = Za2 * i0;
-        if (first) { k0 = rtx * ka; k1 = rty * ka; break; }
-        v0 = z0 + Za0 * ka; v1 = z1 + Za1 * ka; v2 = z2 + Za2 * ka;
-        V00 = S00 + Za0 * Ka0; V01 = S01 + Za0 * Ka1; V02 = M02 + Za0 * Ka2;
-        V11 = S11 + Za1 * Ka1; V12 = M12 + Za1 * Ka2; V22 = Z22 + Za2 * Ka2;
-        k0 = rtx * ka; k1 = rty * ka; K00 = rtx * Ka0; K01 = rtx * Ka1; K02 = rtx * Ka2; K10 = rty * Ka0; K11 = rty * Ka1; K12 = rty * Ka2;
-        break;
-      }
-      case RC_W: {
-        const T hbb = Z22 + c22;
-        const T i0 = -ric_rcp(ric_pivot(hbb, ric_max((T)1e-6 * ric_abs(hbb), (T)1e-30)));
-        k2 = q2 * i0;
-        if (first) break;
-        K20 = M02 * i0; K21 = M12 * i0; K22 = Z22 * i0;
-        v0 = z0 + M02 * k2; v1 = z1 + M12 * k2; v2 = z2 + Z22 * k2;
-        V00 = S00 + M02 * K20; V01 = S01 + M02 * K21; V02 = M02 + M02 * K22;
-        V11 = S11 + M12 * K21; V12 = M12 + M12 * K22; V22 = Z22 + Z22 * K22;
-        break;
-      }
-      case RC_KINK:
-        k0 = e0; k1 = e1; k2 = e2;
-        if (first) break;
-        v0 = z0 + S00 * k0 + S01 * k1 + M02 * k2;
-        v1 = z1 + S01 * k0 + S11 * k1 + M12 * k2;
-        v2 = z2 + Z02 * k0 + Z12 * k1 + Z22 * k2;
-        V00 = S00; V01 = S01; V02 = M02; V11 = S11; V12 = M12; V22 = Z22;
-        break;
-      default:
-        v0 = z0; v1 = z1; v2 = z2;
-        V00 = S00; V01 = S01; V02 = M02; V11 = S11; V12 = M12; V22 = Z22;
-        break;
-    }
+    RicGains<T> g;
+    riccati_stage<T>(q0, q1, q2, q3, q4, q5, q6, sx, i == n - 1, first, wts, val, g);
     if (lane == 0) {
       ric_f4* G4 = reinterpret_cast<ric_f4*>(RS + kRicStage * i + RS_GAIN);
-      G4[0] = ric_f4{(float)K00, (float)K01, (float)K02, (float)K10};
-      G4[1] = ric_f4{(float)K11, (float)K12, (float)K20, (float)K21};
-      G4[2] = ric_f4{(float)K22, (float)k0, (float)k1, (float)k2};
-      AMODE[4 * i + 3] = tokink ? 1 : 0;
+      G4[0] = ric_f4{(float)g.K00, (float)g.K01, (float)g.K02, (float)g.K10};
+      G4[1] = ric_f4{(float)g.K11, (float)g.K12, (float)g.K20, (float)g.K21};
+      G4[2] = ric_f4{(float)g.K22, (float)g.k0, (float)g.k1, (float)g.k2};
+      AMODE[4 * i + 3] = g.tokink ? 1 : 0;
     }
   }
   WAVE_SYNC();
@@ -303,6 +339,89 @@
   WAVE_SYNC();
 }
 
+template <typename T, int kFew>
+__device__ __forceinline__ void riccati_direction_few(const SolveArgs& a, const Ctx& c, double* L, int lane, double& dl0,
+                                                      double& dl1, double& dl2, int& near) {
+  static_assert(kFew >= 1 && kFew <= 4, "unrolled sweeps");
+  constexpr int kInRegs = kFew < kRicGainsInRegisters ? kFew : kRicGainsInRegisters;
+  const DevParams& p = a.p;
+  float* RS = static_cast<float*>(__builtin_assume_aligned(reinterpret_cast<float*>(L + a.lds.ric), 16));
+  const float* ARTF = reinterpret_cast<const float*>(L + a.lds.rt);
+  const RicWeights<T> wts{(T)(2.0 * p.wt_n), (T)(2.0 * p.wo_n), (T)(2.0 * p.wterm_o), (T)((p.wc_n * p.wc_n) / (p.dt * p.dt))};
+  RicValue<T> val;
+  RicGains<T> g[kFew];
+  T px[kFew], py[kFew];
+  bool tok[kFew];
+#pragma unroll
+  for (int i = kFew - 1; i >= 0; --i) {
+    const ric_f4* R4 = reinterpret_cast<const ric_f4*>(RS + kRicStage * i);
+    const ric_f4 r0 = R4[0], r1 = R4[1], r2 = R4[2], r3 = R4[3], r4 = R4[4], r5 = R4[5], r6 = R4[6];
+    const T sx = (T)ARTF[2 * i + 1];
+    px[i] = r0.x; py[i] = r0.y;
+    riccati_stage<T>(r0, r1, r2, r3, r4, r5, r6, sx, i == kFew - 1, i == 0, wts, val, g[i]);
+    tok[i] = g[i].tokink;
+    if (i >= kInRegs && lane == 0) {
+      ric_f4* G4 = reinterpret_cast<ric_f4*>(RS + kRicStage * i + RS_GAIN);
+      G4[0] = ric_f4{(float)g[i].K00, (float)g[i].K01, (float)g[i].K02, (float)g[i].K10};
+      G4[1] = ric_f4{(float)g[i].K11, (float)g[i].K12, (float)g[i].K20, (float)g[i].K21};
+      G4[2] = ric_f4{(float)g[i].K22, (float)g[i].k0, (float)g[i].k1, (float)g[i].k2};
+    }
+  }
+  if (kFew > kInRegs) {
+    WAVE_SYNC();
+#pragma unroll
+    for (int i = kInRegs; i < kFew; ++i) {
+      const ric_f4* G4 = reinterpret_cast<const ric_f4*>(RS + kRicStage * i + RS_GAIN);
+      const ric_f4 g0 = G4[0], g1 = G4[1], g2 = G4[2];
+      g[i].K00 = (T)g0.x; g[i].K01 = (T)g0.y; g[i].K02 = (T)g0.z; g[i].K10 = (T)g0.w;
+      g[i].K11 = (T)g1.x; g[i].K12 = (T)g1.y; g[i].K20 = (T)g1.z; g[i].K21 = (T)g1.w;
+      g[i].K22 = (T)g2.x; g[i].k0 = (T)g2.y; g[i].k1 = (T)g2.z; g[i].k2 = (T)g2.w;
+    }
+  }
+  const bool on = lane < kFew;
+  const int ls = on ? lane : 0;
+  const float* rs = RS + kRicStage * ls;
+  int* am = reinterpret_cast<int*>(L + a.lds.mode) + 4 * ls;
+  const double* u = L + a.lds.u + 3 * ls;
+  const double cs = rs[RS_CS], sn = rs[RS_SN];
+  const int am0 = am[0], am1 = am[1], am2 = am[2];
+  const double nx = L[a.lds.nx + ls], ny = L[a.lds.ny + ls];
+  const double u0 = u[0], u1 = u[1], u2 = u[2];
+  T z0 = (T)0.0, z1 = (T)0.0, z2 = (T)0.0;
+  T mw0 = (T)0.0, mw1 = (T)0.0, mw2 = (T)0.0;
+  bool tokink = false;
+#pragma unroll
+  for (int i = 0; i < kFew; ++i) {
+    const T w0 = (T)g[i].k0 + (T)g[i].K00 * z0 + (T)g[i].K01 * z1 + (T)g[i].K02 * z2;
+    const T w1 = (T)g[i].k1 + (T)g[i].K10 * z0 + (T)g[i].K11 * z1 + (T)g[i].K12 * z2;
+    const T w2f = (T)g[i].k2 + (T)g[i].K20 * z0 + (T)g[i].K21 * z1 + (T)g[i].K22 * z2;
+    if (lane == i) { mw0 = w0; mw1 = w1; mw2 = w2f; tokink = tok[i]; }
+    const T e0 = z0 + w0, e1 = z1 + w1, e2 = z2 + w2f;
+    z0 = ric_fma(-(T)py[i], e2, e0); z1 = ric_fma((T)px[i], e2, e1); z2 = e2;
+  }
+  dl0 = 0.0; dl1 = 0.0; dl2 = 0.0; near = 0;
+  if (on) {
+    double* d = L + a.lds.d + 3 * lane;
+    am[3] = tokink ? 1 : 0;
+    if (tokink) {
+      dl0 = c.v0 - u0; dl1 = c.v1 - u1; dl2 = c.v2 - u2;
+    } else {
+      const double idt = rcp_fast(a.p.dt);
+      const double w0 = (double)mw0, w1 = (double)mw1, w2 = (double)mw2;
+      double d0 = (cs * w0 + sn * w1) * idt, d1 = (-sn * w0 + cs * w1) * idt;
+      const int mode = am2 ? 2 : am0;
+      if (mode == 1) {
+        const double dot = d0 * nx + d1 * ny;
+        d0 -= dot * nx; d1 -= dot * ny;
+      } else if (mode == 2) { d0 = 0.0; d1 = 0.0; }
+      dl0 = d0; dl1 = d1; dl2 = (am2 || (am1 & 1)) ? 0.0 : w2 * idt;
+    }
+    d[0] = dl0; d[1] = dl1; d[2] = dl2;
+    near = am2;
+  }
+  WAVE_SYNC();
+}
+
 template <bool kTame, bool kCovered, int kFew, bool kWantTerm>
 __device__ __forceinline__ bool riccati_free_space_trial(const SolveArgs& a, const Ctx& c, double* L, int n, int lane,
                                                          double alpha_now, double f, double& fb, double& cterm) {
diff --git a/neo_mpc_planner2_amd/csrc/tangent_cone.h b/neo_mpc_planner2_amd/csrc/tangent_cone.h
--- a/neo_mpc_planner2_amd/csrc/tangent_cone.h
+++ b/neo_mpc_planner2_amd/csrc/tangent_cone.h
@@ -10,8 +10,9 @@
 
 constexpr int kNewtonRecord = 13;
 
-template <bool kTame, bool kNewton, bool kRiccati>
-__device__ __forceinline__ bool tangent_cone_pass(const SolveArgs& a, const Ctx& c, double* L, double kink_radius, int lane, int n) {
+template <bool kTame, bool kNewton, bool kRiccati, bool kLocal = false>
+__device__ __forceinline__ bool tangent_cone_pass(const SolveArgs& a, const Ctx& c, double* L, double kink_radius, int lane, int n,
+                                                  StageLocal& sl) {
   constexpr bool kSecond = kNewton || kRiccati;
   const DevParams& p = a.p;
   const double* u = L + a.lds.u;
@@ -25,8 +26,8 @@
   float* ARTF = reinterpret_cast<float*>(L + a.lds.rt);
   bool my_corner = false;
   for (int i = lane; i < n; i += kLanes) {
-    const double u0 = u[3 * i], u1 = u[3 * i + 1], u2 = u[3 * i + 2];
-    const double g0 = gs[3 * i], g1 = gs[3 * i + 1], g2 = gs[3 * i + 2];
+    const double u0 = kLocal ? sl.u0 : u[3 * i], u1 = kLocal ? sl.u1 : u[3 * i + 1], u2 = kLocal ? sl.u2 : u[3 * i + 2];
+    const double g0 = kLocal ? sl.gs0 : gs[3 * i], g1 = kLocal ? sl.gs1 : gs[3 * i + 1], g2 = kLocal ? sl.gs2 : gs[3 * i + 2];
     const double e0 = u0 - c.v0, e1 = u1 - c.v1, e2 = u2 - c.v2;
     const double ne2 = e0 * e0 + e1 * e1 + e2 * e2;
     const double ine = ne2 > 0.0 ? rsq_fast(ne2) : 0.0;
@@ -92,6 +93,10 @@
         for (int k = 0; k < kNewtonRecord; ++k) NB[kNewtonRecord * i + k] = 0.0f;
       }
       if (kRiccati) ARTF[2 * i] = 0.0f;
+      if (kLocal) {
+        sl.gs0 = r0; sl.gs1 = r1; sl.gs2 = s2; sl.gt0 = 0.0; sl.gt1 = 0.0; sl.gt2 = 0.0;
+        sl.nx = 0.0; sl.ny = 0.0; sl.mode = 0; sl.wfroz = 0; sl.near = at_rest; sl.k2 = 0.0f;
+      }
       continue;
     }
     gr[3 * i] = r0; gr[3 * i + 1] = r1; gr[3 * i + 2] = wfroz ? 0.0 : t2;
@@ -100,7 +105,9 @@
       my_corner = my_corner || (mslot != 0 && (u0 - p.lo[0] <= room || p.hi[0] - u0 <= room)) ||
                   (mslot != 1 && (u1 - p.lo[1] <= room || p.hi[1] - u1 <= room)) || (mslot != 2 && nvv2 >= rin * rin);
     }
-    ANX[i] = mnx; ANY[i] = mny; AMODE[4 * i] = mode; AMODE[4 * i + 1] = wfroz | ((mode == 1 && mslot == 2) ? 2 : 0); AMODE[4 * i + 2] = 0;
+    const int wslot = wfroz | ((mode == 1 && mslot == 2) ? 2 : 0);
+    ANX[i] = mnx; ANY[i] = mny; AMODE[4 * i] = mode; AMODE[4 * i + 1] = wslot; AMODE[4 * i + 2] = 0;
+    if (kLocal) { sl.gt0 = t0; sl.gt1 = t1; sl.gt2 = t2; sl.nx = mnx; sl.ny = mny; sl.mode = mode; sl.wfroz = wslot; sl.near = 0; }
     if (kNewton) {
       float* nb = NB + kNewtonRecord * i;
       nb[0] = mode == 0 ? 1.0f : mode == 1 ? (float)(1.0 - mnx * mnx) : 0.0f;
@@ -120,7 +127,11 @@
       nb[7] = c01; nb[8] = c11; nb[9] = c12;
       nb[10] = c02; nb[11] = c12; nb[12] = c22;
     }
-    if (kRiccati) ARTF[2 * i] = (mode == 1 && mslot == 2) ? (float)(mlam * rcp_fast(p.r)) : 0.0f;
+    if (kRiccati) {
+      const float k2 = (mode == 1 && mslot == 2) ? (float)(mlam * rcp_fast(p.r)) : 0.0f;
+      ARTF[2 * i] = k2;
+      if (kLocal) sl.k2 = k2;
+    }
   }
   return my_corner;
 }
```

Result: faster. 28.75 million, median of 6 (+16.4%).
